# linkedin/spark-tfrecord

Hardware: AMD Instinct MI355X
Metric: rows/sec read+write (1M-row Example round-trip) (higher is better)
Workload: dtype wire(int64/float32/bytes); 1 GPU; model=Example{id:int64, ints:Int64List[8], floats:FloatList[16], tokens:BytesList[2]}, global_batch=1000000, parallelism=dp1, rows_per_rank=1000000, engine=gpu, storage=/dev/shm, crc_verify=True

## Files before the change

csrc/hip/kernels.hip:

```cpp

#include <hip/hip_runtime.h>
#include <pybind11/pybind11.h>
#include <pybind11/stl.h>
#include <rocprim/rocprim.hpp>

#include <fcntl.h>
#include <sys/mman.h>
#include <sys/stat.h>
#include <unistd.h>

#include <cstdint>
#include <map>
#include <mutex>
#include <stdexcept>
#include <string>
#include <vector>

#include "../codec_core.h"

namespace py = pybind11;
using namespace tfrec;

#define HIP_CHECK(expr)                                                          \
  do {                                                                           \
    hipError_t _e = (expr);                                                      \
    if (_e != hipSuccess)                                                        \
      throw std::runtime_error(std::string("HIP error: ") +                      \
                               hipGetErrorString(_e) + " at " __FILE__ ":" +     \
                               std::to_string(__LINE__));                        \
  } while (0)

namespace {

constexpr int kBlock = 256;

__device__ inline void stage_crc_tables(uint32_t (*lds)[256]) {
  const uint32_t* src = &kCrcTables.t[0][0];
  uint32_t* dst = &lds[0][0];
  for (int i = threadIdx.x; i < 8 * 256; i += blockDim.x) dst[i] = src[i];
  __syncthreads();
}

__device__ inline void set_err(int32_t* err, int32_t code, i64 r) {
  err[0] = code;
  i64 v = r + 1;
  atomicMax(&err[1], v > 0x7FFFFFFF ? (int32_t)0x7FFFFFFF : (int32_t)v);
}


__global__ void crc_verify_kernel(const u8* __restrict__ data,
                                  const i64* __restrict__ off,
                                  const i64* __restrict__ len, i64 R,
                                  unsigned long long* err_out) {
  __shared__ uint32_t tab[8][256];
  stage_crc_tables(tab);
  for (i64 r = blockIdx.x * (i64)blockDim.x + threadIdx.x; r < R;
       r += (i64)gridDim.x * blockDim.x) {
    const u8* h = data + off[r] - 12;
    u32 len_crc, data_crc;
    __builtin_memcpy(&len_crc, h + 8, 4);
    __builtin_memcpy(&data_crc, h + 12 + len[r], 4);
    bool ok = mask_crc(crc32c_sw(h, 8, 0, tab)) == len_crc &&
              mask_crc(crc32c_sw(h + 12, (size_t)len[r], 0, tab)) == data_crc;
    if (!ok) atomicMin(err_out, (unsigned long long)(r + 1));
  }
}


static_assert(sizeof(FieldStat) == 48, "FieldStat layout shared with Python");

__global__ void scan_records_kernel(const u8* __restrict__ data,
                                    const i64* __restrict__ off,
                                    const i64* __restrict__ len, i64 R, int32_t fmt,
                                    const u8* __restrict__ schema_blob, int F,
                                    FieldStat* __restrict__ stats,
                                    int32_t* __restrict__ err,
                                    unsigned long long* crc_err) {
  __shared__ uint32_t tab[8][256];
  if (crc_err) stage_crc_tables(tab);
  SchemaView schema = schema_view(schema_blob);
  for (i64 r = blockIdx.x * (i64)blockDim.x + threadIdx.x; r < R;
       r += (i64)gridDim.x * blockDim.x) {
    FieldStat* st = stats + r * F;
    for (int f = 0; f < F; ++f) field_stat_clear(&st[f]);
    int32_t rc;
    if (crc_err) {
      u32 payload_crc = 0;
      rc = scan_record_fused(data, off[r], len[r], fmt, schema, st,
                             &payload_crc, tab);
      if (rc == ERR_RETRY_UNFUSED) {
        for (int f = 0; f < F; ++f) field_stat_clear(&st[f]);
        rc = scan_record(data, off[r], len[r], fmt, schema, st);
        payload_crc = crc32c_sw(data + off[r], (size_t)len[r], 0, tab);
      }
      if (rc != ERR_OK)
        payload_crc = crc32c_sw(data + off[r], (size_t)len[r], 0, tab);
      const u8* h = data + off[r] - 12;
      u32 len_crc, data_crc;
      __builtin_memcpy(&len_crc, h + 8, 4);
      __builtin_memcpy(&data_crc, h + 12 + len[r], 4);
      bool ok = mask_crc(crc32c_sw(h, 8, 0, tab)) == len_crc &&
                mask_crc(payload_crc) == data_crc;
      if (!ok) atomicMin(crc_err, (unsigned long long)(r + 1));
    } else {
      rc = scan_record(data, off[r], len[r], fmt, schema, st);
    }
    if (rc != ERR_OK) set_err(err, rc, r);
    for (int f = 0; f < F; ++f)
      if (st[f].err != ERR_OK) set_err(err, st[f].err, r);
  }
}


struct DevFieldDst {
  int32_t kind;
  int32_t is_seq;
  i64* i64_vals;
  float* f32_vals;
  u8* bytes_data;
  i64* elem_len;
  i64* sub_count;
  const i64* val_base;
  const i64* byte_base;
  const i64* list_base;
};

__global__ void extract_fields_kernel(const u8* __restrict__ data, i64 R, int F,
                                      const FieldStat* __restrict__ stats,
                                      const DevFieldDst* __restrict__ metas,
                                      int32_t* __restrict__ err) {
  i64 total = R * F;
  for (i64 idx = blockIdx.x * (i64)blockDim.x + threadIdx.x; idx < total;
       idx += (i64)gridDim.x * blockDim.x) {
    i64 r = idx / F;
    int f = (int)(idx - r * F);
    const DevFieldDst& m = metas[f];
    const FieldStat& st = stats[r * F + f];
    DecodeDst dst{m.i64_vals, m.f32_vals, m.bytes_data, m.elem_len, m.sub_count};
    int32_t rc = extract_field(data, st.pos, st.len, m.kind, m.is_seq, dst,
                               m.val_base ? m.val_base[r] : 0,
                               m.byte_base ? m.byte_base[r] : 0,
                               m.list_base ? m.list_base[r] : 0);
    if (rc != ERR_OK) set_err(err, rc, r);
  }
}



__global__ void size_records_kernel(const FieldColumn* __restrict__ cols,
                                    const u8* __restrict__ schema_blob, int32_t fmt,
                                    i64 R, i64* __restrict__ psize) {
  SchemaView schema = schema_view(schema_blob);
  for (i64 r = blockIdx.x * (i64)blockDim.x + threadIdx.x; r < R;
       r += (i64)gridDim.x * blockDim.x) {
    psize[r] = record_payload_size(cols, schema, fmt, r) + kFrameOverhead;
  }
}

__global__ void emit_records_kernel(const FieldColumn* __restrict__ cols,
                                    const u8* __restrict__ schema_blob, int32_t fmt,
                                    i64 r0, i64 R, const i64* __restrict__ frame_off,
                                    u8* __restrict__ file,
                                    int32_t* __restrict__ err) {
  __shared__ uint32_t tab[8][256];
  stage_crc_tables(tab);
  SchemaView schema = schema_view(schema_blob);
  for (i64 r = r0 + blockIdx.x * (i64)blockDim.x + threadIdx.x; r < R;
       r += (i64)gridDim.x * blockDim.x) {
    i64 payload = (frame_off[r + 1] - frame_off[r]) - kFrameOverhead;
    u8* o = file + frame_off[r] + 12;
    u32 crc = 0;
    i64 emitted = emit_record_payload_fused(o, cols, schema, fmt, r, &crc,
                                            tab);
    if (emitted != payload) set_err(err, ERR_OVERFLOW, r);
    write_frame_header_footer_crc(file, frame_off[r], payload, crc, tab);
  }
}


constexpr i64 kWaveRecordBytes = 8 << 10;

__device__ inline u32 crc32c_wave(const u8* p, i64 n,
                                  const uint32_t (*tab)[256]) {
  int lane = threadIdx.x & 63;
  i64 chunk = (n + 63) / 64;
  if (chunk < 64) chunk = 64;
  i64 s = (i64)lane * chunk;
  i64 e = s + chunk < n ? s + chunk : n;
  u32 my = (s < e) ? crc32c_sw(p + s, (size_t)(e - s), 0, tab) : 0;
  u32 acc = __shfl(my, 0);
  if (chunk < n) {
    u32 op = crc32c_shift_elem((u64)chunk);
    for (int i = 1; i < 64; ++i) {
      i64 si = (i64)i * chunk;
      if (si >= n) break;
      u32 ci = __shfl(my, i);
      i64 li = (si + chunk < n ? chunk : n - si);
      acc = (li == chunk) ? (crc_gfmul(acc, op) ^ ci)
                          : crc32c_combine_fast(acc, ci, (u64)li);
    }
  }
  return acc;
}

__device__ inline void copy_wave(u8* d, const u8* s, i64 n) {
  int lane = threadIdx.x & 63;
  i64 i = (i64)lane * 8;
  for (; i + 8 <= n; i += 64 * 8) {
    u64 w;
    __builtin_memcpy(&w, s + i, 8);
    __builtin_memcpy(d + i, &w, 8);
  }
  i64 tail = n & ~((i64)7);
  for (i64 b = tail + lane; b < n; b += 64) d[b] = s[b];
}

__global__ void crc_verify_wave_kernel(const u8* __restrict__ data,
                                       const i64* __restrict__ off,
                                       const i64* __restrict__ len, i64 R,
                                       unsigned long long* err_out) {
  __shared__ uint32_t tab[8][256];
  stage_crc_tables(tab);
  i64 wave = (blockIdx.x * (i64)blockDim.x + threadIdx.x) / 64;
  i64 nwaves = ((i64)gridDim.x * blockDim.x) / 64;
  for (i64 r = wave; r < R; r += nwaves) {
    const u8* h = data + off[r] - 12;
    u32 payload = crc32c_wave(h + 12, len[r], tab);
    if ((threadIdx.x & 63) == 0) {
      u32 len_crc, data_crc;
      __builtin_memcpy(&len_crc, h + 8, 4);
      __builtin_memcpy(&data_crc, h + 12 + len[r], 4);
      bool ok = mask_crc(crc32c_sw(h, 8, 0, tab)) == len_crc &&
                mask_crc(payload) == data_crc;
      if (!ok) atomicMin(err_out, (unsigned long long)(r + 1));
    }
  }
}

__global__ void frame_bytes_wave_kernel(const u8* __restrict__ src,
                                        const i64* __restrict__ elem_off,
                                        const i64* __restrict__ frame_off, i64 R,
                                        u8* __restrict__ file) {
  __shared__ uint32_t tab[8][256];
  stage_crc_tables(tab);
  i64 wave = (blockIdx.x * (i64)blockDim.x + threadIdx.x) / 64;
  i64 nwaves = ((i64)gridDim.x * blockDim.x) / 64;
  for (i64 r = wave; r < R; r += nwaves) {
    i64 n = elem_off[r + 1] - elem_off[r];
    const u8* s = src + elem_off[r];
    u8* d = file + frame_off[r] + 12;
    copy_wave(d, s, n);
    u32 crc = crc32c_wave(s, n, tab);
    if ((threadIdx.x & 63) == 0)
      write_frame_header_footer_crc(file, frame_off[r], n, crc, tab);
  }
}

__global__ void gather_payloads_wave_kernel(const u8* __restrict__ data,
                                            const i64* __restrict__ off,
                                            const i64* __restrict__ len,
                                            const i64* __restrict__ dst_off,
                                            i64 R, u8* __restrict__ out) {
  i64 wave = (blockIdx.x * (i64)blockDim.x + threadIdx.x) / 64;
  i64 nwaves = ((i64)gridDim.x * blockDim.x) / 64;
  for (i64 r = wave; r < R; r += nwaves)
    copy_wave(out + dst_off[r], data + off[r], len[r]);
}


__device__ inline i64 wave_incl_scan(i64 v) {
  int lane = threadIdx.x & 63;
  for (int d = 1; d < 64; d <<= 1) {
    i64 y = __shfl_up(v, d);
    if (lane >= d) v += y;
  }
  return v;
}

__device__ inline i64 wave_extract_i64_packed(const u8* __restrict__ p, i64 n,
                                              i64* __restrict__ out, i64 base) {
  int lane = threadIdx.x & 63;
  i64 chunk = (n + 63) / 64;
  i64 lo = (i64)lane * chunk;
  i64 hi = lo + chunk < n ? lo + chunk : n;
  i64 cnt = 0;
  for (i64 i = lo; i < hi; ++i) cnt += !(p[i] & 0x80);
  i64 incl = wave_incl_scan(cnt);
  i64 excl = incl - cnt;
  i64 total = __shfl(incl, 63);
  i64 q = lo;
  i64 pre = 0;
  if (lo > 0 && lo < hi) {
    if (p[lo - 1] & 0x80) {
      while (q < hi && (p[q] & 0x80)) ++q;
      if (q < hi) {
        ++q;
        pre = 1;
      }
    }
  }
  i64 idx = base + excl + pre;
  while (q < hi) {
    u64 v = 0;
    int shift = 0;
    i64 j = q;
    while (j < n && shift < 70) {
      u8 b = p[j++];
      v |= (u64)(b & 0x7F) << shift;
      shift += 7;
      if (!(b & 0x80)) break;
    }
    out[idx++] = (i64)v;
    q = j;
  }
  return total;
}

__device__ inline int32_t extract_list_body_wave(const u8* __restrict__ p,
                                                 const u8* end, int32_t kind,
                                                 const DecodeDst& dst, i64* vi,
                                                 i64* bi) {
  int lane = threadIdx.x & 63;
  while (p < end) {
    u64 tag;
    p = read_varint(p, end, &tag);
    if (!p) return ERR_BAD_VARINT;
    u32 fieldno = (u32)(tag >> 3), wt = (u32)(tag & 7);
    if (fieldno != 1) {
      p = skip_field(p, end, wt);
      if (!p) return ERR_TRUNCATED;
      continue;
    }
    if (kind == KIND_BYTES) {
      u64 len;
      p = read_varint(p, end, &len);
      if (!p || (u64)(end - p) < len) return ERR_TRUNCATED;
      copy_wave(dst.bytes_data + *bi, p, (i64)len);
      if (lane == 0) dst.elem_len[*vi] = (i64)len;
      *bi += (i64)len;
      *vi += 1;
      p += len;
    } else if (kind == KIND_FLOAT) {
      if (wt == 2) {
        u64 len;
        p = read_varint(p, end, &len);
        if (!p || (u64)(end - p) < len) return ERR_TRUNCATED;
        u64 nv = len / 4;
        copy_wave((u8*)(dst.f32_vals + *vi), p, (i64)(nv * 4));
        *vi += (i64)nv;
        p += len;
      } else {
        if (end - p < 4) return ERR_TRUNCATED;
        if (lane == 0) {
          float v;
          __builtin_memcpy(&v, p, 4);
          dst.f32_vals[*vi] = v;
        }
        (*vi)++;
        p += 4;
      }
    } else {
      if (wt == 2) {
        u64 len;
        p = read_varint(p, end, &len);
        if (!p || (u64)(end - p) < len) return ERR_TRUNCATED;
        *vi += wave_extract_i64_packed(p, (i64)len, dst.i64_vals, *vi);
        p += len;
      } else {
        u64 v;
        p = read_varint(p, end, &v);
        if (!p) return ERR_BAD_VARINT;
        if (lane == 0) dst.i64_vals[*vi] = (i64)v;
        (*vi)++;
      }
    }
  }
  return ERR_OK;
}

__device__ inline int32_t extract_feature_body_wave(const u8* __restrict__ p,
                                                    const u8* end, int32_t kind,
                                                    const DecodeDst& dst,
                                                    i64* vi, i64* bi) {
  while (p < end) {
    u64 tag;
    p = read_varint(p, end, &tag);
    if (!p) return ERR_BAD_VARINT;
    u32 fieldno = (u32)(tag >> 3), wt = (u32)(tag & 7);
    if (fieldno >= 1 && fieldno <= 3 && wt == 2) {
      u64 len;
      p = read_varint(p, end, &len);
      if (!p || (u64)(end - p) < len) return ERR_TRUNCATED;
      int32_t rc = extract_list_body_wave(p, p + len, kind, dst, vi, bi);
      if (rc != ERR_OK) return rc;
      p += len;
    } else {
      p = skip_field(p, end, wt);
      if (!p) return ERR_TRUNCATED;
    }
  }
  return ERR_OK;
}

__device__ inline int32_t extract_field_wave(const u8* __restrict__ data,
                                             i64 pos, i64 len, int32_t kind,
                                             int32_t is_seq, const DecodeDst& dst,
                                             i64 val_base, i64 byte_base,
                                             i64 list_base) {
  if (pos < 0) return ERR_OK;
  int lane = threadIdx.x & 63;
  const u8* p = data + pos;
  const u8* end = p + len;
  i64 vi = val_base;
  i64 bi = byte_base;
  if (!is_seq) return extract_feature_body_wave(p, end, kind, dst, &vi, &bi);
  i64 li = list_base;
  while (p < end) {
    u64 tag;
    p = read_varint(p, end, &tag);
    if (!p) return ERR_BAD_VARINT;
    u32 fieldno = (u32)(tag >> 3), wt = (u32)(tag & 7);
    if (fieldno == 1 && wt == 2) {
      u64 flen;
      p = read_varint(p, end, &flen);
      if (!p || (u64)(end - p) < flen) return ERR_TRUNCATED;
      i64 v_before = vi;
      int32_t rc = extract_feature_body_wave(p, p + flen, kind, dst, &vi, &bi);
      if (rc != ERR_OK) return rc;
      if (lane == 0) dst.sub_count[li] = vi - v_before;
      ++li;
      p += flen;
    } else {
      p = skip_field(p, end, wt);
      if (!p) return ERR_TRUNCATED;
    }
  }
  return ERR_OK;
}

__global__ void scan_records_wave_kernel(const u8* __restrict__ data,
                                         const i64* __restrict__ off,
                                         const i64* __restrict__ len, i64 R,
                                         int32_t fmt,
                                         const u8* __restrict__ schema_blob,
                                         int F, FieldStat* __restrict__ stats,
                                         int32_t* __restrict__ err,
                                         unsigned long long* crc_err) {
  __shared__ uint32_t tab[8][256];
  stage_crc_tables(tab);
  SchemaView schema = schema_view(schema_blob);
  i64 wave = (blockIdx.x * (i64)blockDim.x + threadIdx.x) / 64;
  i64 nwaves = ((i64)gridDim.x * blockDim.x) / 64;
  int lane = threadIdx.x & 63;
  for (i64 r = wave; r < R; r += nwaves) {
    if (lane == 0) {
      FieldStat* st = stats + r * F;
      for (int f = 0; f < F; ++f) field_stat_clear(&st[f]);
      int32_t rc = scan_record(data, off[r], len[r], fmt, schema, st);
      if (rc != ERR_OK) set_err(err, rc, r);
      for (int f = 0; f < F; ++f)
        if (st[f].err != ERR_OK) set_err(err, st[f].err, r);
    }
    if (crc_err) {
      const u8* h = data + off[r] - 12;
      u32 payload = crc32c_wave(h + 12, len[r], tab);
      if (lane == 0) {
        u32 len_crc, data_crc;
        __builtin_memcpy(&len_crc, h + 8, 4);
        __builtin_memcpy(&data_crc, h + 12 + len[r], 4);
        bool ok = mask_crc(crc32c_sw(h, 8, 0, tab)) == len_crc &&
                  mask_crc(payload) == data_crc;
        if (!ok) atomicMin(crc_err, (unsigned long long)(r + 1));
      }
    }
  }
}

__global__ void extract_fields_wave_kernel(const u8* __restrict__ data, i64 R,
                                           int F,
                                           const FieldStat* __restrict__ stats,
                                           const DevFieldDst* __restrict__ metas,
                                           int32_t* __restrict__ err) {
  i64 total = R * F;
  i64 wave = (blockIdx.x * (i64)blockDim.x + threadIdx.x) / 64;
  i64 nwaves = ((i64)gridDim.x * blockDim.x) / 64;
  for (i64 idx = wave; idx < total; idx += nwaves) {
    i64 r = idx / F;
    int f = (int)(idx - r * F);
    const DevFieldDst& m = metas[f];
    const FieldStat& st = stats[r * F + f];
    DecodeDst dst{m.i64_vals, m.f32_vals, m.bytes_data, m.elem_len, m.sub_count};
    int32_t rc = extract_field_wave(data, st.pos, st.len, m.kind, m.is_seq, dst,
                                    m.val_base ? m.val_base[r] : 0,
                                    m.byte_base ? m.byte_base[r] : 0,
                                    m.list_base ? m.list_base[r] : 0);
    if (rc != ERR_OK && (threadIdx.x & 63) == 0) set_err(err, rc, r);
  }
}


__device__ inline i64 wave_emit_i64_packed(u8* __restrict__ o,
                                           const i64* __restrict__ vals,
                                           i64 v0, i64 v1) {
  int lane = threadIdx.x & 63;
  i64 n = v1 - v0;
  i64 chunk = (n + 63) / 64;
  i64 lo = v0 + (i64)lane * chunk;
  i64 hi = lo + chunk < v1 ? lo + chunk : v1;
  i64 sz = 0;
  for (i64 v = lo; v < hi; ++v) sz += varint_size((u64)vals[v]);
  i64 incl = wave_incl_scan(sz);
  u8* q = o + (incl - sz);
  for (i64 v = lo; v < hi; ++v) q = write_varint(q, (u64)vals[v]);
  return __shfl(incl, 63);
}

struct WaveCur {
  u8* base;
  i64 pos;
};

__device__ inline void wvc_put(WaveCur& w, u8 b) {
  if ((threadIdx.x & 63) == 0) w.base[w.pos] = b;
  w.pos += 1;
}

__device__ inline void wvc_varint(WaveCur& w, u64 v) {
  if ((threadIdx.x & 63) == 0) write_varint(w.base + w.pos, v);
  w.pos += varint_size(v);
}

__device__ inline void wvc_bytes(WaveCur& w, const u8* s, i64 n) {
  copy_wave(w.base + w.pos, s, n);
  w.pos += n;
}

__device__ inline void wvc_list_body(WaveCur& w, const FieldColumn& c, i64 v0,
                                     i64 v1) {
  if (c.kind == KIND_FLOAT) {
    i64 n = v1 - v0;
    if (n) {
      wvc_put(w, 0x0A);
      wvc_varint(w, (u64)(4 * n));
      wvc_bytes(w, (const u8*)(c.f32_vals + v0), 4 * n);
    }
  } else if (c.kind == KIND_INT64) {
    i64 packed = 0;
    for (i64 v = v0; v < v1; ++v) packed += varint_size((u64)c.i64_vals[v]);
    if (packed) {
      wvc_put(w, 0x0A);
      wvc_varint(w, (u64)packed);
      w.pos += wave_emit_i64_packed(w.base + w.pos, c.i64_vals, v0, v1);
    }
  } else {
    for (i64 v = v0; v < v1; ++v) {
      i64 b0 = c.elem_off[v];
      i64 blen = c.elem_off[v + 1] - b0;
      wvc_put(w, 0x0A);
      wvc_varint(w, (u64)blen);
      wvc_bytes(w, c.bytes_data + b0, blen);
    }
  }
}

__device__ inline void wvc_feature_body(WaveCur& w, const FieldColumn& c,
                                        i64 v0, i64 v1) {
  i64 body = list_body_size(c, v0, v1);
  wvc_put(w, (u8)((c.kind << 3) | 2));
  wvc_varint(w, (u64)body);
  wvc_list_body(w, c, v0, v1);
}

__device__ inline void wvc_features_entry(WaveCur& w, const FieldColumn& c,
                                          const SchemaView& s, int f, i64 v0,
                                          i64 v1) {
  i64 fb = feature_body_size(c, v0, v1);
  i64 klen = s.name_len(f);
  wvc_put(w, 0x0A);
  wvc_varint(w, (u64)klen);
  wvc_bytes(w, s.name(f), klen);
  wvc_put(w, 0x12);
  wvc_varint(w, (u64)fb);
  wvc_feature_body(w, c, v0, v1);
}

__device__ inline void wvc_feature_lists_entry(WaveCur& w, const FieldColumn& c,
                                               const SchemaView& s, int f,
                                               i64 r) {
  i64 flb = feature_list_body_size(c, r);
  i64 klen = s.name_len(f);
  wvc_put(w, 0x0A);
  wvc_varint(w, (u64)klen);
  wvc_bytes(w, s.name(f), klen);
  wvc_put(w, 0x12);
  wvc_varint(w, (u64)flb);
  for (i64 j = c.list_off[r]; j < c.list_off[r + 1]; ++j) {
    i64 fb = feature_body_size(c, c.sub_off[j], c.sub_off[j + 1]);
    wvc_put(w, 0x0A);
    wvc_varint(w, (u64)fb);
    wvc_feature_body(w, c, c.sub_off[j], c.sub_off[j + 1]);
  }
}

__device__ inline i64 emit_record_payload_wave(u8* o, const FieldColumn* cols,
                                               const SchemaView& s, int32_t fmt,
                                               i64 r) {
  i64 ctx_body = 0, fl_body = 0;
  for (int f = 0; f < s.nfields; ++f) {
    const FieldColumn& c = cols[f];
    if (!c.presence[r]) continue;
    if (!c.is_seq) {
      i64 e = features_entry_size(c, s, f, c.row_off[r], c.row_off[r + 1]);
      ctx_body += 1 + varint_size((u64)e) + e;
    } else {
      i64 e = feature_lists_entry_size(c, s, f, r);
      fl_body += 1 + varint_size((u64)e) + e;
    }
  }
  WaveCur w{o, 0};
  auto emit_ctx = [&]() {
    for (int f = 0; f < s.nfields; ++f) {
      const FieldColumn& c = cols[f];
      if (!c.presence[r] || c.is_seq) continue;
      i64 e = features_entry_size(c, s, f, c.row_off[r], c.row_off[r + 1]);
      wvc_put(w, 0x0A);
      wvc_varint(w, (u64)e);
      wvc_features_entry(w, c, s, f, c.row_off[r], c.row_off[r + 1]);
    }
  };
  auto emit_fl = [&]() {
    for (int f = 0; f < s.nfields; ++f) {
      const FieldColumn& c = cols[f];
      if (!c.presence[r] || !c.is_seq) continue;
      i64 e = feature_lists_entry_size(c, s, f, r);
      wvc_put(w, 0x0A);
      wvc_varint(w, (u64)e);
      wvc_feature_lists_entry(w, c, s, f, r);
    }
  };
  if (fmt == FMT_EXAMPLE) {
    wvc_put(w, 0x0A);
    wvc_varint(w, (u64)ctx_body);
    emit_ctx();
  } else {
    if (ctx_body) {
      wvc_put(w, 0x0A);
      wvc_varint(w, (u64)ctx_body);
      emit_ctx();
    }
    wvc_put(w, 0x12);
    wvc_varint(w, (u64)fl_body);
    emit_fl();
  }
  return w.pos;
}

__global__ void emit_records_wave_kernel(const FieldColumn* __restrict__ cols,
                                         const u8* __restrict__ schema_blob,
                                         int32_t fmt, i64 r0, i64 R,
                                         const i64* __restrict__ frame_off,
                                         u8* __restrict__ file,
                                         int32_t* __restrict__ err) {
  __shared__ uint32_t tab[8][256];
  stage_crc_tables(tab);
  SchemaView schema = schema_view(schema_blob);
  i64 wave = (blockIdx.x * (i64)blockDim.x + threadIdx.x) / 64;
  i64 nwaves = ((i64)gridDim.x * blockDim.x) / 64;
  int lane = threadIdx.x & 63;
  for (i64 r = r0 + wave; r < R; r += nwaves) {
    i64 payload = (frame_off[r + 1] - frame_off[r]) - kFrameOverhead;
    u8* o = file + frame_off[r] + 12;
    i64 emitted = emit_record_payload_wave(o, cols, schema, fmt, r);
    if (emitted != payload && lane == 0) set_err(err, ERR_OVERFLOW, r);
    __threadfence_block();
    u32 crc = crc32c_wave(o, payload, tab);
    if (lane == 0)
      write_frame_header_footer_crc(file, frame_off[r], payload, crc, tab);
  }
}

__global__ void frame_bytes_kernel(const u8* __restrict__ src,
                                   const i64* __restrict__ elem_off,
                                   const i64* __restrict__ frame_off, i64 R,
                                   u8* __restrict__ file) {
  __shared__ uint32_t tab[8][256];
  stage_crc_tables(tab);
  for (i64 r = blockIdx.x * (i64)blockDim.x + threadIdx.x; r < R;
       r += (i64)gridDim.x * blockDim.x) {
    i64 n = elem_off[r + 1] - elem_off[r];
    WriteCur w;
    wcur_init(w, file + frame_off[r] + 12, tab);
    wcur_bytes(w, src + elem_off[r], n);
    u32 crc = wcur_finish(w);
    write_frame_header_footer_crc(file, frame_off[r], n, crc, tab);
  }
}

__device__ inline u32 crc8b_reg(u64 w, const uint32_t (*tab)[256]) {
  w ^= 0xFFFFFFFFull;
  u32 c = tab[7][w & 0xFF] ^ tab[6][(w >> 8) & 0xFF] ^ tab[5][(w >> 16) & 0xFF] ^
          tab[4][(w >> 24) & 0xFF] ^ tab[3][(w >> 32) & 0xFF] ^
          tab[2][(w >> 40) & 0xFF] ^ tab[1][(w >> 48) & 0xFF] ^
          tab[0][(w >> 56) & 0xFF];
  return ~c;
}

constexpr int kPosPerLane = 16;

template <typename F>
__device__ inline void eval_frame_chunk(const u8* __restrict__ data,
                                        const u64* __restrict__ wdata, i64 N,
                                        i64 c, i64 pos_start, i64 pos_end,
                                        const uint32_t (*tab)[256], F&& f) {
  i64 p0 = c * kPosPerLane;
  i64 w0 = p0 >> 3;
  u64 w[4];
  if (p0 + 32 <= N) {
#pragma unroll
    for (int j = 0; j < 4; ++j) w[j] = wdata[w0 + j];
  } else {
#pragma unroll
    for (int j = 0; j < 4; ++j) {
      u64 v = 0;
      i64 boff = (w0 + j) * 8;
      for (int b = 0; b < 8 && boff + b < N; ++b)
        v |= (u64)data[boff + b] << (8 * b);
      w[j] = v;
    }
  }
#pragma unroll
  for (int k = 0; k < kPosPerLane; ++k) {
    i64 i = p0 + k;
    if (i + 16 > N || i >= pos_end) break;
    if (i < pos_start) continue;
    constexpr int _ppl = kPosPerLane;
    static_assert(_ppl == 16, "index math below assumes 16 positions");
    const int wi = k >> 3;
    const int sh = (k & 7) * 8;
    u64 len = (sh == 0) ? w[wi] : (w[wi] >> sh) | (w[wi + 1] << (64 - sh));
    if (len > (u64)(N - i) - 16) continue;
    const int wi2 = (k + 8) >> 3;
    const int sh2 = sh;
    u64 hi = (sh2 == 0) ? w[wi2]
                        : (w[wi2] >> sh2) | (w[wi2 + 1] << (64 - sh2));
    u32 want = (u32)hi;
    if (mask_crc(crc8b_reg(len, tab)) != want) continue;
    f(i, (i64)len);
  }
}

template <bool EMIT>
__global__ void frame_scan_pass_kernel(const u8* __restrict__ data, i64 N,
                                       i64 pos_start, i64 pos_end,
                                       i64 block_base,
                                       i64* __restrict__ block_data,
                                       i64* __restrict__ cand_pos,
                                       i64* __restrict__ cand_len) {
  __shared__ uint32_t tab[8][256];
  __shared__ unsigned int cnt[256];
  stage_crc_tables(tab);
  const u64* wdata = reinterpret_cast<const u64*>(data);
  i64 c_lo = pos_start / kPosPerLane;
  i64 c_hi = (pos_end + kPosPerLane - 1) / kPosPerLane;
  i64 c = c_lo + (i64)blockIdx.x * blockDim.x + threadIdx.x;
  unsigned int my = 0;
  if (c < c_hi)
    eval_frame_chunk(data, wdata, N, c, pos_start, pos_end, tab,
                     [&](i64, i64) { ++my; });
  cnt[threadIdx.x] = my;
  __syncthreads();
  if (!EMIT) {
    for (int off = blockDim.x / 2; off; off >>= 1) {
      if ((int)threadIdx.x < off) cnt[threadIdx.x] += cnt[threadIdx.x + off];
      __syncthreads();
    }
    if (threadIdx.x == 0) block_data[block_base + blockIdx.x] = (i64)cnt[0];
    return;
  }
  for (int off = 1; off < (int)blockDim.x; off <<= 1) {
    unsigned int v = (int)threadIdx.x >= off ? cnt[threadIdx.x - off] : 0;
    __syncthreads();
    cnt[threadIdx.x] += v;
    __syncthreads();
  }
  i64 slot = block_data[block_base + blockIdx.x] + (i64)(cnt[threadIdx.x] - my);
  if (c < c_hi)
    eval_frame_chunk(data, wdata, N, c, pos_start, pos_end, tab,
                     [&](i64 i, i64 len) {
                       cand_pos[slot] = i;
                       cand_len[slot] = len;
                       ++slot;
                     });
}


struct InferSlot {
  unsigned long long hash;
  long long nameref;
  long long code;
};
static_assert(sizeof(InferSlot) == 24, "layout shared with Python [S,3] i64");

__device__ inline u64 fnv1a64(const u8* s, u64 n) {
  u64 h = 1469598103934665603ull;
  for (u64 i = 0; i < n; ++i) h = (h ^ s[i]) * 1099511628211ull;
  return h ? h : 1ull;
}

constexpr int kLdsInfer = 64;

struct LdsInferSlot {
  unsigned long long hash;
  long long nameref;
  unsigned int code;
};

__device__ inline bool lds_infer_merge(LdsInferSlot* ltab, u64 hash,
                                       long long nameref, int code) {
  int idx = (int)(hash % (u64)kLdsInfer);
  for (int probe = 0; probe < kLdsInfer; ++probe) {
    LdsInferSlot& s = ltab[idx];
    unsigned long long seen =
        atomicCAS(&s.hash, 0ull, (unsigned long long)hash);
    if (seen == 0ull) s.nameref = nameref;
    if (seen == 0ull || seen == hash) {
      atomicMax(&s.code, (unsigned int)code);
      return true;
    }
    idx = (idx + 1) % kLdsInfer;
  }
  return false;
}

__device__ inline bool infer_slot_merge(InferSlot* table, int lo, int half,
                                        u64 hash, long long nameref, int code) {
  int idx = lo + (int)(hash % (u64)half);
  for (int probe = 0; probe < half; ++probe) {
    InferSlot& s = table[idx];
    unsigned long long seen =
        atomicCAS(&s.hash, 0ull, (unsigned long long)hash);
    if (seen == 0ull) s.nameref = nameref;
    if (seen == 0ull || seen == hash) {
      atomicMax((unsigned long long*)&s.code, (unsigned long long)code);
      return true;
    }
    idx = (idx + 1 - lo) % half + lo;
  }
  return false;
}

__device__ inline int32_t infer_features_body_dev(const u8* data, const u8* p,
                                                  const u8* end, bool seq,
                                                  LdsInferSlot* ltab,
                                                  InferSlot* table, int nslots) {
  int half = nslots / 2;
  int lo = seq ? half : 0;
  while (p < end) {
    u64 tag;
    p = read_varint(p, end, &tag);
    if (!p) return ERR_BAD_VARINT;
    u32 fieldno = (u32)(tag >> 3), wt = (u32)(tag & 7);
    if (fieldno != 1 || wt != 2) {
      p = skip_field(p, end, wt);
      if (!p) return ERR_TRUNCATED;
      continue;
    }
    u64 entry_len;
    p = read_varint(p, end, &entry_len);
    if (!p || (u64)(end - p) < entry_len) return ERR_TRUNCATED;
    const u8* ep = p;
    const u8* ee = p + entry_len;
    p = ee;
    const u8* key = nullptr;
    u64 key_len = 0;
    const u8* val = nullptr;
    u64 val_len = 0;
    while (ep < ee) {
      u64 etag;
      ep = read_varint(ep, ee, &etag);
      if (!ep) return ERR_BAD_VARINT;
      u32 efn = (u32)(etag >> 3), ewt = (u32)(etag & 7);
      if (efn == 1 && ewt == 2) {
        ep = read_varint(ep, ee, &key_len);
        if (!ep || (u64)(ee - ep) < key_len) return ERR_TRUNCATED;
        key = ep;
        ep += key_len;
      } else if (efn == 2 && ewt == 2) {
        ep = read_varint(ep, ee, &val_len);
        if (!ep || (u64)(ee - ep) < val_len) return ERR_TRUNCATED;
        val = ep;
        ep += val_len;
      } else {
        ep = skip_field(ep, ee, ewt);
        if (!ep) return ERR_TRUNCATED;
      }
    }
    if (!key) continue;
    int code = 0;
    if (val) {
      if (!seq) {
        int32_t kf = 0;
        i64 nvals = 0, nbytes = 0;
        int32_t rc = scan_feature_body(val, val + val_len, -1, &kf, &nvals, &nbytes);
        if (rc != ERR_OK) return rc;
        if (kf != 0 && nvals > 0) code = (4 - kf) + (nvals > 1 ? 3 : 0);
      } else {
        const u8* lp = val;
        const u8* le = val + val_len;
        int kind_seen = 0;
        while (lp < le) {
          u64 ltag;
          lp = read_varint(lp, le, &ltag);
          if (!lp) return ERR_BAD_VARINT;
          u32 lfn = (u32)(ltag >> 3), lwt = (u32)(ltag & 7);
          if (lfn == 1 && lwt == 2) {
            u64 flen;
            lp = read_varint(lp, le, &flen);
            if (!lp || (u64)(le - lp) < flen) return ERR_TRUNCATED;
            int32_t kf = 0;
            i64 nvals = 0, nbytes = 0;
            int32_t rc = scan_feature_body(lp, lp + flen, -1, &kf, &nvals, &nbytes);
            if (rc != ERR_OK) return rc;
            if (kf) {
              int r = 4 - kf;
              kind_seen = kind_seen > r ? kind_seen : r;
            }
            lp += flen;
          } else {
            lp = skip_field(lp, le, lwt);
            if (!lp) return ERR_TRUNCATED;
          }
        }
        if (kind_seen) code = 6 + kind_seen;
      }
    }
    if (key_len > 0xFFFF) return ERR_NAME_TOO_LONG;
    long long nameref = ((long long)(key - data) << 16) | (long long)key_len;
    u64 hash = fnv1a64(key, key_len);
    if (!lds_infer_merge(ltab, hash, nameref, code) &&
        !infer_slot_merge(table, lo, half, hash, nameref, code))
      return ERR_OVERFLOW;
  }
  return ERR_OK;
}

__global__ void infer_codes_kernel(const u8* __restrict__ data,
                                   const i64* __restrict__ off,
                                   const i64* __restrict__ len, i64 R, int32_t fmt,
                                   InferSlot* __restrict__ table, int nslots,
                                   int32_t* __restrict__ err) {
  __shared__ LdsInferSlot lctx[kLdsInfer];
  __shared__ LdsInferSlot lseq[kLdsInfer];
  for (int i = threadIdx.x; i < kLdsInfer; i += blockDim.x) {
    lctx[i].hash = 0;
    lctx[i].code = 0;
    lseq[i].hash = 0;
    lseq[i].code = 0;
  }
  __syncthreads();
  for (i64 r = blockIdx.x * (i64)blockDim.x + threadIdx.x; r < R;
       r += (i64)gridDim.x * blockDim.x) {
    const u8* p = data + off[r];
    const u8* end = p + len[r];
    while (p < end) {
      u64 tag;
      const u8* np = read_varint(p, end, &tag);
      if (!np) {
        set_err(err, ERR_BAD_VARINT, r);
        break;
      }
      p = np;
      u32 fieldno = (u32)(tag >> 3), wt = (u32)(tag & 7);
      bool is_features = fieldno == 1;
      bool is_fl = (fmt == FMT_SEQUENCE && fieldno == 2);
      if ((is_features || is_fl) && wt == 2) {
        u64 blen;
        p = read_varint(p, end, &blen);
        if (!p || (u64)(end - p) < blen) {
          set_err(err, ERR_TRUNCATED, r);
          break;
        }
        int32_t rc = infer_features_body_dev(data, p, p + blen, is_fl,
                                             is_fl ? lseq : lctx, table, nslots);
        if (rc != ERR_OK) {
          set_err(err, rc, r);
          break;
        }
        p += blen;
      } else {
        p = skip_field(p, end, wt);
        if (!p) {
          set_err(err, ERR_TRUNCATED, r);
          break;
        }
      }
    }
  }
  __syncthreads();
  int half = nslots / 2;
  for (int i = threadIdx.x; i < kLdsInfer; i += blockDim.x) {
    if (lctx[i].hash &&
        !infer_slot_merge(table, 0, half, lctx[i].hash, lctx[i].nameref,
                          (int)lctx[i].code))
      err[0] = ERR_OVERFLOW;
    if (lseq[i].hash &&
        !infer_slot_merge(table, half, half, lseq[i].hash, lseq[i].nameref,
                          (int)lseq[i].code))
      err[0] = ERR_OVERFLOW;
  }
}

__global__ void gather_payloads_kernel(const u8* __restrict__ data,
                                       const i64* __restrict__ off,
                                       const i64* __restrict__ len,
                                       const i64* __restrict__ dst_off, i64 R,
                                       u8* __restrict__ out) {
  for (i64 r = blockIdx.x * (i64)blockDim.x + threadIdx.x; r < R;
       r += (i64)gridDim.x * blockDim.x) {
    const u8* s = data + off[r];
    u8* d = out + dst_off[r];
    i64 n = len[r];
    i64 i = 0;
    for (; i + 8 <= n; i += 8) {
      u64 w;
      __builtin_memcpy(&w, s + i, 8);
      __builtin_memcpy(d + i, &w, 8);
    }
    for (; i < n; ++i) d[i] = s[i];
  }
}


inline int grid_for(i64 n) {
  i64 blocks = (n + kBlock - 1) / kBlock;
  if (blocks > 8192) blocks = 8192;
  if (blocks < 1) blocks = 1;
  return (int)blocks;
}

void gpu_crc_verify(uintptr_t data, uintptr_t off, uintptr_t len, i64 R,
                    uintptr_t err_out, uintptr_t stream, i64 avg_bytes) {
  if (avg_bytes > kWaveRecordBytes) {
    hipLaunchKernelGGL(crc_verify_wave_kernel, dim3(grid_for(R * 64)),
                       dim3(kBlock), 0, (hipStream_t)stream, (const u8*)data,
                       (const i64*)off, (const i64*)len, R,
                       (unsigned long long*)err_out);
  } else {
    hipLaunchKernelGGL(crc_verify_kernel, dim3(grid_for(R)), dim3(kBlock), 0,
                       (hipStream_t)stream, (const u8*)data, (const i64*)off,
                       (const i64*)len, R, (unsigned long long*)err_out);
  }
  HIP_CHECK(hipGetLastError());
}

void gpu_scan_records(uintptr_t data, uintptr_t off, uintptr_t len, i64 R,
                      int32_t fmt, uintptr_t schema_blob, int F, uintptr_t stats,
                      uintptr_t err, uintptr_t crc_err, uintptr_t stream,
                      i64 avg_bytes) {
  if (avg_bytes > kWaveRecordBytes) {
    hipLaunchKernelGGL(scan_records_wave_kernel, dim3(grid_for(R * 64)),
                       dim3(kBlock), 0, (hipStream_t)stream, (const u8*)data,
                       (const i64*)off, (const i64*)len, R, fmt,
                       (const u8*)schema_blob, F, (FieldStat*)stats,
                       (int32_t*)err, (unsigned long long*)crc_err);
  } else {
    hipLaunchKernelGGL(scan_records_kernel, dim3(grid_for(R)), dim3(kBlock), 0,
                       (hipStream_t)stream, (const u8*)data, (const i64*)off,
                       (const i64*)len, R, fmt, (const u8*)schema_blob, F,
                       (FieldStat*)stats, (int32_t*)err,
                       (unsigned long long*)crc_err);
  }
  HIP_CHECK(hipGetLastError());
}

void gpu_extract_fields(uintptr_t data, i64 R, int F, uintptr_t stats,
                        py::list metas, uintptr_t meta_dev, uintptr_t err,
                        uintptr_t stream, i64 avg_bytes) {
  std::vector<DevFieldDst> host_metas(F);
  for (int f = 0; f < F; ++f) {
    py::dict d = metas[f].cast<py::dict>();
    DevFieldDst& m = host_metas[f];
    m.kind = d["kind"].cast<int32_t>();
    m.is_seq = d["is_seq"].cast<int32_t>();
    m.i64_vals = (i64*)d["i64_vals"].cast<uintptr_t>();
    m.f32_vals = (float*)d["f32_vals"].cast<uintptr_t>();
    m.bytes_data = (u8*)d["bytes_data"].cast<uintptr_t>();
    m.elem_len = (i64*)d["elem_len"].cast<uintptr_t>();
    m.sub_count = (i64*)d["sub_count"].cast<uintptr_t>();
    m.val_base = (const i64*)d["val_base"].cast<uintptr_t>();
    m.byte_base = (const i64*)d["byte_base"].cast<uintptr_t>();
    m.list_base = (const i64*)d["list_base"].cast<uintptr_t>();
  }
  HIP_CHECK(hipMemcpyAsync((void*)meta_dev, host_metas.data(),
                           sizeof(DevFieldDst) * F, hipMemcpyHostToDevice,
                           (hipStream_t)stream));
  if (avg_bytes > kWaveRecordBytes) {
    hipLaunchKernelGGL(extract_fields_wave_kernel, dim3(grid_for(R * F * 64)),
                       dim3(kBlock), 0, (hipStream_t)stream, (const u8*)data,
                       R, F, (const FieldStat*)stats,
                       (const DevFieldDst*)meta_dev, (int32_t*)err);
  } else {
    hipLaunchKernelGGL(extract_fields_kernel, dim3(grid_for(R * F)),
                       dim3(kBlock), 0, (hipStream_t)stream, (const u8*)data,
                       R, F, (const FieldStat*)stats,
                       (const DevFieldDst*)meta_dev, (int32_t*)err);
  }
  HIP_CHECK(hipGetLastError());
}

size_t gpu_devcols_bytes(int F) { return sizeof(FieldColumn) * (size_t)F; }

void fill_devcols(py::list cols, std::vector<FieldColumn>& out) {
  int F = (int)cols.size();
  out.resize(F);
  for (int f = 0; f < F; ++f) {
    py::dict d = cols[f].cast<py::dict>();
    FieldColumn& c = out[f];
    c.kind = d["kind"].cast<int32_t>();
    c.is_seq = d["is_seq"].cast<int32_t>();
    c.presence = (const u8*)d["presence"].cast<uintptr_t>();
    c.row_off = (const i64*)d["row_off"].cast<uintptr_t>();
    c.list_off = (const i64*)d["list_off"].cast<uintptr_t>();
    c.sub_off = (const i64*)d["sub_off"].cast<uintptr_t>();
    c.elem_off = (const i64*)d["elem_off"].cast<uintptr_t>();
    c.bytes_data = (const u8*)d["values_bytes"].cast<uintptr_t>();
    c.i64_vals = (const i64*)d["values_i64"].cast<uintptr_t>();
    c.f32_vals = (const float*)d["values_f32"].cast<uintptr_t>();
  }
}

void gpu_size_records(py::list cols, uintptr_t cols_dev, uintptr_t schema_blob,
                      int32_t fmt, i64 R, uintptr_t psize, uintptr_t stream) {
  static thread_local std::vector<FieldColumn> host_cols;
  fill_devcols(cols, host_cols);
  HIP_CHECK(hipMemcpyAsync((void*)cols_dev, host_cols.data(),
                           sizeof(FieldColumn) * host_cols.size(),
                           hipMemcpyHostToDevice, (hipStream_t)stream));
  hipLaunchKernelGGL(size_records_kernel, dim3(grid_for(R)), dim3(kBlock), 0,
                     (hipStream_t)stream, (const FieldColumn*)cols_dev,
                     (const u8*)schema_blob, fmt, R, (i64*)psize);
  HIP_CHECK(hipGetLastError());
}

void gpu_emit_records(uintptr_t cols_dev, uintptr_t schema_blob, int32_t fmt,
                      i64 r0, i64 R, uintptr_t frame_off, uintptr_t file,
                      uintptr_t err, uintptr_t stream, i64 avg_bytes) {
  if (avg_bytes > kWaveRecordBytes) {
    hipLaunchKernelGGL(emit_records_wave_kernel, dim3(grid_for((R - r0) * 64)),
                       dim3(kBlock), 0, (hipStream_t)stream,
                       (const FieldColumn*)cols_dev, (const u8*)schema_blob,
                       fmt, r0, R, (const i64*)frame_off, (u8*)file,
                       (int32_t*)err);
  } else {
    hipLaunchKernelGGL(emit_records_kernel, dim3(grid_for(R - r0)),
                       dim3(kBlock), 0, (hipStream_t)stream,
                       (const FieldColumn*)cols_dev, (const u8*)schema_blob,
                       fmt, r0, R, (const i64*)frame_off, (u8*)file,
                       (int32_t*)err);
  }
  HIP_CHECK(hipGetLastError());
}

void gpu_frame_bytes(uintptr_t src, uintptr_t elem_off, uintptr_t frame_off, i64 R,
                     uintptr_t file, uintptr_t stream, i64 avg_bytes) {
  if (avg_bytes > kWaveRecordBytes) {
    hipLaunchKernelGGL(frame_bytes_wave_kernel, dim3(grid_for(R * 64)),
                       dim3(kBlock), 0, (hipStream_t)stream, (const u8*)src,
                       (const i64*)elem_off, (const i64*)frame_off, R,
                       (u8*)file);
  } else {
    hipLaunchKernelGGL(frame_bytes_kernel, dim3(grid_for(R)), dim3(kBlock), 0,
                       (hipStream_t)stream, (const u8*)src, (const i64*)elem_off,
                       (const i64*)frame_off, R, (u8*)file);
  }
  HIP_CHECK(hipGetLastError());
}

i64 gpu_frame_scan_blocks(i64 pos_start, i64 pos_end) {
  i64 c_lo = pos_start / kPosPerLane;
  i64 c_hi = (pos_end + kPosPerLane - 1) / kPosPerLane;
  i64 n = c_hi - c_lo;
  return (n + kBlock - 1) / kBlock;
}

void gpu_frame_scan_count(uintptr_t data, i64 N, i64 pos_start, i64 pos_end,
                          i64 block_base, uintptr_t block_counts,
                          uintptr_t stream) {
  i64 B = gpu_frame_scan_blocks(pos_start, pos_end);
  if (B <= 0) return;
  hipLaunchKernelGGL(frame_scan_pass_kernel<false>, dim3((uint32_t)B),
                     dim3(kBlock), 0, (hipStream_t)stream, (const u8*)data, N,
                     pos_start, pos_end, block_base, (i64*)block_counts,
                     nullptr, nullptr);
  HIP_CHECK(hipGetLastError());
}

void gpu_frame_scan_emit(uintptr_t data, i64 N, i64 pos_start, i64 pos_end,
                         i64 block_base, uintptr_t block_off,
                         uintptr_t cand_pos, uintptr_t cand_len,
                         uintptr_t stream) {
  i64 B = gpu_frame_scan_blocks(pos_start, pos_end);
  if (B <= 0) return;
  hipLaunchKernelGGL(frame_scan_pass_kernel<true>, dim3((uint32_t)B),
                     dim3(kBlock), 0, (hipStream_t)stream, (const u8*)data, N,
                     pos_start, pos_end, block_base, (i64*)block_off,
                     (i64*)cand_pos, (i64*)cand_len);
  HIP_CHECK(hipGetLastError());
}

void gpu_infer_codes(uintptr_t data, uintptr_t off, uintptr_t len, i64 R,
                     int32_t fmt, uintptr_t table, int nslots, uintptr_t err,
                     uintptr_t stream) {
  hipLaunchKernelGGL(infer_codes_kernel, dim3(grid_for(R)), dim3(kBlock), 0,
                     (hipStream_t)stream, (const u8*)data, (const i64*)off,
                     (const i64*)len, R, fmt, (InferSlot*)table, nslots,
                     (int32_t*)err);
  HIP_CHECK(hipGetLastError());
}

void gpu_gather_payloads(uintptr_t data, uintptr_t off, uintptr_t len,
                         uintptr_t dst_off, i64 R, uintptr_t out,
                         uintptr_t stream, i64 avg_bytes) {
  if (avg_bytes > kWaveRecordBytes) {
    hipLaunchKernelGGL(gather_payloads_wave_kernel, dim3(grid_for(R * 64)),
                       dim3(kBlock), 0, (hipStream_t)stream, (const u8*)data,
                       (const i64*)off, (const i64*)len, (const i64*)dst_off,
                       R, (u8*)out);
  } else {
    hipLaunchKernelGGL(gather_payloads_kernel, dim3(grid_for(R)), dim3(kBlock),
                       0, (hipStream_t)stream, (const u8*)data,
                       (const i64*)off, (const i64*)len, (const i64*)dst_off,
                       R, (u8*)out);
  }
  HIP_CHECK(hipGetLastError());
}


struct StridedLoadI64 {
  const i64* p;
  i64 stride;
  __host__ __device__ i64 operator()(i64 i) const { return p[i * stride]; }
};

size_t gpu_scan_temp_bytes(i64 n) {
  size_t bytes = 0;
  auto it = rocprim::make_transform_iterator(
      rocprim::make_counting_iterator<i64>(0), StridedLoadI64{nullptr, 1});
  (void)rocprim::inclusive_scan(nullptr, bytes, it, (i64*)nullptr, (size_t)n,
                                rocprim::plus<i64>());
  return bytes;
}


struct Seg3 {
  i64 v0, v1, v2;
  u32 flag;
};

struct Seg3Combine {
  __host__ __device__ Seg3 operator()(const Seg3& a, const Seg3& b) const {
    if (b.flag) return b;
    return Seg3{a.v0 + b.v0, a.v1 + b.v1, a.v2 + b.v2, a.flag};
  }
};

struct Seg3Load {
  const i64* stats;
  i64 R;
  int F;
  __host__ __device__ Seg3 operator()(i64 idx) const {
    i64 f = idx / R;
    i64 r = idx - f * R;
    const i64* st = stats + (r * F + f) * 6;
    return Seg3{st[2], st[3], st[4], r == 0 ? 1u : 0u};
  }
};

struct Seg3OutRef {
  i64* o0;
  i64* o1;
  i64* o2;
  __host__ __device__ Seg3OutRef& operator=(const Seg3& v) {
    *o0 = v.v0;
    *o1 = v.v1;
    *o2 = v.v2;
    return *this;
  }
};

struct Seg3OutIt {
  using value_type = Seg3;
  using reference = Seg3OutRef;
  using pointer = Seg3OutRef*;
  using difference_type = i64;
  using iterator_category = std::random_access_iterator_tag;
  i64* b0;
  i64* b1;
  i64* b2;
  i64 R;
  i64 pos;
  __host__ __device__ Seg3OutRef operator*() const { return (*this)[0]; }
  __host__ __device__ Seg3OutRef operator[](i64 k) const {
    i64 idx = pos + k;
    i64 f = idx / R;
    i64 r = idx - f * R;
    i64 at = f * (R + 1) + r + 1;
    return Seg3OutRef{b0 + at, b1 + at, b2 + at};
  }
  __host__ __device__ Seg3OutIt operator+(i64 k) const {
    return Seg3OutIt{b0, b1, b2, R, pos + k};
  }
  __host__ __device__ Seg3OutIt& operator+=(i64 k) {
    pos += k;
    return *this;
  }
  __host__ __device__ Seg3OutIt& operator++() {
    ++pos;
    return *this;
  }
};

size_t gpu_stat_scan_temp_bytes(i64 R, int F) {
  size_t bytes = 0;
  auto in = rocprim::make_transform_iterator(
      rocprim::make_counting_iterator<i64>(0), Seg3Load{nullptr, R, F});
  Seg3OutIt out{nullptr, nullptr, nullptr, R, 0};
  (void)rocprim::inclusive_scan(nullptr, bytes, in, out, (size_t)(R * F),
                                Seg3Combine());
  return bytes;
}

void gpu_stat_scans(uintptr_t temp, size_t temp_bytes, uintptr_t stats, i64 R,
                    int F, uintptr_t val_base, uintptr_t byte_base,
                    uintptr_t list_base, uintptr_t stream) {
  auto s = (hipStream_t)stream;
  if (R <= 0 || F <= 0) return;
  auto in = rocprim::make_transform_iterator(
      rocprim::make_counting_iterator<i64>(0),
      Seg3Load{(const i64*)stats, R, F});
  Seg3OutIt out{(i64*)val_base, (i64*)byte_base, (i64*)list_base, R, 0};
  size_t tb = temp_bytes;
  HIP_CHECK(rocprim::inclusive_scan((void*)temp, tb, in, out,
                                    (size_t)(R * F), Seg3Combine(), s));
}

void gpu_excl_sum_strided(uintptr_t temp, size_t temp_bytes, uintptr_t in,
                          i64 stride, uintptr_t out, i64 n, uintptr_t stream) {
  auto s = (hipStream_t)stream;
  HIP_CHECK(hipMemsetAsync((void*)out, 0, sizeof(i64), s));
  if (n <= 0) return;
  auto it = rocprim::make_transform_iterator(
      rocprim::make_counting_iterator<i64>(0), StridedLoadI64{(const i64*)in, stride});
  size_t tb = temp_bytes;
  hipError_t e = rocprim::inclusive_scan((void*)temp, tb, it, (i64*)out + 1,
                                         (size_t)n, rocprim::plus<i64>(), s);
  HIP_CHECK(e);
}


struct MappedFile {
  void* ptr = nullptr;
  size_t n = 0;
  dev_t dev = 0;
  ino_t ino = 0;
  bool pinned = false;
  bool writable = false;
};

std::map<std::string, MappedFile> g_mmap_cache;
std::mutex g_mmap_mu;
size_t g_mmap_bytes = 0;
constexpr size_t kMmapCacheCap = 4ull << 30;

void drop_mapping_locked(const std::string& key) {
  auto it = g_mmap_cache.find(key);
  if (it == g_mmap_cache.end()) return;
  if (it->second.pinned) {
    (void)hipDeviceSynchronize();
    (void)hipHostUnregister(it->second.ptr);
  }
  munmap(it->second.ptr, it->second.n);
  g_mmap_bytes -= it->second.n;
  g_mmap_cache.erase(it);
}

void sweep_stale_locked() {
  for (auto it = g_mmap_cache.begin(); it != g_mmap_cache.end();) {
    struct stat st {};
    bool live = stat(it->first.c_str(), &st) == 0 &&
                st.st_dev == it->second.dev && st.st_ino == it->second.ino &&
                (size_t)st.st_size >= it->second.n;
    if (live) {
      ++it;
    } else {
      auto key = it->first;
      ++it;
      drop_mapping_locked(key);
    }
  }
}

py::tuple file_mmap_pinned(const std::string& path, i64 n, bool writable) {
  if (n <= 0) return py::make_tuple((uintptr_t)0, true);
  std::lock_guard<std::mutex> lk(g_mmap_mu);
  sweep_stale_locked();
  int flags = writable ? (O_RDWR | O_CREAT) : O_RDWR;
  int fd = ::open(path.c_str(), flags, 0644);
  bool rdonly = false;
  if (fd < 0 && !writable) {
    fd = ::open(path.c_str(), O_RDONLY);
    rdonly = true;
  }
  if (fd < 0)
    throw std::runtime_error("open failed: " + path + ": " + strerror(errno));
  struct stat st {};
  if (fstat(fd, &st) != 0) {
    ::close(fd);
    throw std::runtime_error("stat failed: " + path);
  }
  auto it = g_mmap_cache.find(path);
  if (it != g_mmap_cache.end()) {
    MappedFile& m = it->second;
    if (m.dev == st.st_dev && m.ino == st.st_ino && m.n == (size_t)n &&
        st.st_size >= (off_t)n && (m.writable || !writable)) {
      ::close(fd);
      return py::make_tuple((uintptr_t)m.ptr, m.pinned);
    }
    drop_mapping_locked(path);
  }
  if (writable && st.st_size != (off_t)n && ftruncate(fd, (off_t)n) != 0) {
    int e = errno;
    ::close(fd);
    throw std::runtime_error("ftruncate failed: " + path + ": " + strerror(e));
  }
  if (!writable && st.st_size < (off_t)n) {
    ::close(fd);
    throw std::runtime_error("short file: " + path);
  }
  while (g_mmap_bytes + (size_t)n > kMmapCacheCap && !g_mmap_cache.empty())
    drop_mapping_locked(g_mmap_cache.begin()->first);
  int prot = PROT_READ | ((writable || !rdonly) ? PROT_WRITE : 0);
  void* p = mmap(nullptr, (size_t)n, prot, MAP_SHARED, fd, 0);
  ::close(fd);
  if (p == MAP_FAILED)
    throw std::runtime_error("mmap failed: " + path + ": " + strerror(errno));
  bool pinned = hipHostRegister(p, (size_t)n, hipHostRegisterDefault) == hipSuccess;
  if (!pinned) (void)hipGetLastError();
  MappedFile m{p, (size_t)n, st.st_dev, st.st_ino, pinned,
               writable || !rdonly};
  g_mmap_cache[path] = m;
  g_mmap_bytes += (size_t)n;
  return py::make_tuple((uintptr_t)p, pinned);
}

void file_mmap_drop(const std::string& path) {
  std::lock_guard<std::mutex> lk(g_mmap_mu);
  drop_mapping_locked(path);
}

void file_mmap_sync(const std::string& path) {
  std::lock_guard<std::mutex> lk(g_mmap_mu);
  auto it = g_mmap_cache.find(path);
  if (it != g_mmap_cache.end() && it->second.ptr) {
    if (msync(it->second.ptr, it->second.n, MS_SYNC) != 0)
      throw std::runtime_error("msync failed: " + path + ": " +
                               strerror(errno));
  }
  int fd = ::open(path.c_str(), O_RDONLY);
  if (fd >= 0) {
    (void)fsync(fd);
    ::close(fd);
  }
}


void gpu_memcpy_d2h(uintptr_t dst, uintptr_t src, i64 n, uintptr_t stream) {
  HIP_CHECK(hipMemcpyAsync((void*)dst, (const void*)src, (size_t)n,
                           hipMemcpyDeviceToHost, (hipStream_t)stream));
}

void gpu_memcpy_h2d(uintptr_t dst, uintptr_t src, i64 n, uintptr_t stream) {
  HIP_CHECK(hipMemcpyAsync((void*)dst, (const void*)src, (size_t)n,
                           hipMemcpyHostToDevice, (hipStream_t)stream));
}

}

void register_gpu(py::module_& m) {
  m.def("gpu_device_count", []() {
    int n = 0;
    hipError_t e = hipGetDeviceCount(&n);
    return (e == hipSuccess) ? n : -static_cast<int>(e);
  });
  m.def("gpu_crc_verify", &gpu_crc_verify, py::arg("data"), py::arg("off"),
        py::arg("len"), py::arg("R"), py::arg("err_out"), py::arg("stream"),
        py::arg("avg_bytes") = 0);
  m.def("gpu_scan_records", &gpu_scan_records, py::arg("data"), py::arg("off"),
        py::arg("len"), py::arg("R"), py::arg("fmt"), py::arg("schema_blob"),
        py::arg("F"), py::arg("stats"), py::arg("err"), py::arg("crc_err"),
        py::arg("stream"), py::arg("avg_bytes") = 0);
  m.def("gpu_extract_fields", &gpu_extract_fields, py::arg("data"),
        py::arg("R"), py::arg("F"), py::arg("stats"), py::arg("metas"),
        py::arg("meta_dev"), py::arg("err"), py::arg("stream"),
        py::arg("avg_bytes") = 0);
  m.def("gpu_size_records", &gpu_size_records);
  m.def("gpu_emit_records", &gpu_emit_records, py::arg("cols_dev"),
        py::arg("schema_blob"), py::arg("fmt"), py::arg("r0"), py::arg("R"),
        py::arg("frame_off"), py::arg("file"), py::arg("err"),
        py::arg("stream"), py::arg("avg_bytes") = 0);
  m.def("gpu_frame_bytes", &gpu_frame_bytes, py::arg("src"),
        py::arg("elem_off"), py::arg("frame_off"), py::arg("R"),
        py::arg("file"), py::arg("stream"), py::arg("avg_bytes") = 0);
  m.def("gpu_frame_scan_blocks", &gpu_frame_scan_blocks);
  m.def("gpu_frame_scan_count", &gpu_frame_scan_count);
  m.def("gpu_frame_scan_emit", &gpu_frame_scan_emit);
  m.def("gpu_gather_payloads", &gpu_gather_payloads, py::arg("data"),
        py::arg("off"), py::arg("len"), py::arg("dst_off"), py::arg("R"),
        py::arg("out"), py::arg("stream"), py::arg("avg_bytes") = 0);
  m.def("gpu_infer_codes", &gpu_infer_codes);
  m.def("gpu_scan_temp_bytes", &gpu_scan_temp_bytes);
  m.def("gpu_stat_scan_temp_bytes", &gpu_stat_scan_temp_bytes);
  m.def("gpu_stat_scans", &gpu_stat_scans);
  m.def("gpu_excl_sum_strided", &gpu_excl_sum_strided);
  m.def("file_mmap_pinned", &file_mmap_pinned, py::arg("path"), py::arg("n"),
        py::arg("writable"));
  m.def("file_mmap_drop", &file_mmap_drop);
  m.def("file_mmap_sync", &file_mmap_sync);
  m.def("gpu_memcpy_d2h", &gpu_memcpy_d2h);
  m.def("gpu_memcpy_h2d", &gpu_memcpy_h2d);
  m.def("gpu_devcols_bytes", &gpu_devcols_bytes);
  m.def("gpu_devmeta_bytes", []() { return sizeof(DevFieldDst); });
  m.def("gpu_fieldstat_words", []() { return sizeof(FieldStat) / 8; });
}
```

spark_tfrecord_amd/engine/gpu.py:

```python

from __future__ import annotations

import os
from typing import List, Optional

import numpy as np
import torch

from .. import _native
from ..columnar import RecordBatch, WireColumn, schema_blob, wire_fields
from ..schema import KIND_BYTES, KIND_FLOAT, KIND_INT64, StructType, is_sequence_field, wire_kind_of

FMT = {"Example": _native.FMT_EXAMPLE, "SequenceExample": _native.FMT_SEQUENCE}

_U64_MAX = 0xFFFFFFFFFFFFFFFF


def _stream() -> int:
    return torch.cuda.current_stream().cuda_stream


def _dev(x, dtype, device="cuda") -> torch.Tensor:
    if isinstance(x, torch.Tensor):
        return x.to(device=device, dtype=dtype).contiguous()
    arr = np.ascontiguousarray(x)
    import warnings

    with warnings.catch_warnings():
        warnings.simplefilter("ignore", UserWarning)
        return torch.as_tensor(arr, dtype=dtype).to(device)


def check_native():
    if not getattr(_native, "HAS_GPU_KERNELS", False):
        raise RuntimeError("_native was built without HIP kernels; rebuild "
                           "with build_native.py before using the GPU engine")



import threading as _threading

_pinned_tls = _threading.local()


def pinned_buffer(tag: str, nbytes: int) -> torch.Tensor:
    pool = getattr(_pinned_tls, "pool", None)
    if pool is None:
        pool = _pinned_tls.pool = {}
    buf = pool.get(tag)
    if buf is None or buf.numel() < nbytes:
        cap = max(nbytes, int((buf.numel() if buf is not None else 1 << 20) * 1.5))
        buf = torch.empty(cap, dtype=torch.uint8, pin_memory=True)
        pool[tag] = buf
    return buf


_CHUNK = 64 << 20
_READ_SLICE = int(os.environ.get("TFREC_READ_SLICE", 48 << 20))
_WRITE_SLICES = int(os.environ.get("TFREC_WRITE_SLICES", 8))
_PRESCAN = os.environ.get("TFREC_PRESCAN", "0") == "1"
_SYNC_WRITES = os.environ.get("TFREC_SYNC", "1") != "0"


def read_file_to_device(path: str, device="cuda") -> torch.Tensor:
    import os as _os

    n = _os.path.getsize(path)
    dev_t = torch.empty(max(n, 1), dtype=torch.uint8, device=device)[:n]
    if n:
        ptr, pinned = _native.file_mmap_pinned(path, n, False)
        if pinned:
            _multi_dma(dev_t.data_ptr(), ptr, n, _native.gpu_memcpy_h2d,
                       after_main=True)
            return dev_t
    return _read_file_staged(path, dev_t)


_copy_streams: Optional[list] = None


def _dma_streams() -> list:
    global _copy_streams
    if _copy_streams is None:
        _copy_streams = [torch.cuda.Stream() for _ in range(2)]
    return _copy_streams


def _multi_dma(dst: int, src: int, n: int, fn, after_main: bool):
    streams = _dma_streams()
    main = torch.cuda.current_stream()
    k = min(len(streams), max(1, n // (16 << 20)))
    span = (n + k - 1) // k
    for i in range(k):
        o = i * span
        m = min(span, n - o)
        s = streams[i]
        s.wait_stream(main)
        fn(dst + o, src + o, m, s.cuda_stream)
    if after_main:
        for i in range(k):
            main.wait_stream(streams[i])
    else:
        for i in range(k):
            streams[i].synchronize()


def _read_file_staged(path: str, dev: torch.Tensor) -> torch.Tensor:
    import os as _os

    n = dev.numel()
    buf = pinned_buffer("fread", min(n, 2 * _CHUNK) or 1)
    ev = [torch.cuda.Event(), torch.cuda.Event()]
    fd = _os.open(path, _os.O_RDONLY)
    try:
        pos = 0
        which = 0
        while pos < n:
            m = min(_CHUNK, n - pos)
            ev[which].synchronize()
            _native.pread_parallel(fd, buf.data_ptr() + which * _CHUNK, m, pos)
            dev[pos:pos + m].copy_(buf[which * _CHUNK:which * _CHUNK + m],
                                   non_blocking=True)
            ev[which].record()
            pos += m
            which ^= 1 if n > _CHUNK else 0
    finally:
        _os.close(fd)
    return dev


def device_to_file(img: torch.Tensor, path: str):
    import os as _os

    n = img.numel()
    if n == 0:
        open(path, "wb").close()
        return
    ptr, pinned = _native.file_mmap_pinned(path, n, True)
    if pinned:
        _multi_dma(ptr, img.data_ptr(), n, _native.gpu_memcpy_d2h,
                   after_main=False)
        if _SYNC_WRITES:
            _native.file_mmap_sync(path)
        return
    _write_file_staged(img, path)


def _write_file_staged(img: torch.Tensor, path: str):
    import os as _os

    n = img.numel()
    buf = pinned_buffer("fwrite", min(n, 2 * _CHUNK) or 1)
    ev = [torch.cuda.Event(), torch.cuda.Event()]
    fd = _os.open(path, _os.O_RDWR | _os.O_CREAT, 0o644)
    try:
        pos = 0
        which = 0
        m0 = min(_CHUNK, n)
        if n:
            buf[0:m0].copy_(img[0:m0], non_blocking=True)
            ev[0].record()
        while pos < n:
            m = min(_CHUNK, n - pos)
            nxt = pos + m
            nwhich = which ^ (1 if n > _CHUNK else 0)
            if nxt < n:
                m2 = min(_CHUNK, n - nxt)
                buf[nwhich * _CHUNK:nwhich * _CHUNK + m2].copy_(
                    img[nxt:nxt + m2], non_blocking=True)
                ev[nwhich].record()
            ev[which].synchronize()
            _native.pwrite_parallel(fd, buf.data_ptr() + which * _CHUNK, m, pos)
            pos = nxt
            which = nwhich
        _os.ftruncate(fd, n)
        if _SYNC_WRITES:
            _os.fsync(fd)
    finally:
        _os.close(fd)



_scan_ws = {}


def _scan_workspace(n: int, device) -> torch.Tensor:
    key = (device.index if hasattr(device, "index") else 0)
    need = _native.gpu_scan_temp_bytes(max(n, 1))
    ws = _scan_ws.get(key)
    if ws is None or ws.numel() < need:
        ws = torch.empty(int(need * 2), dtype=torch.uint8, device=device)
        _scan_ws[key] = ws
    return ws


def _excl_sum_into(out_ptr: int, in_ptr: int, stride: int, n: int, device):
    ws = _scan_workspace(n, device)
    _native.gpu_excl_sum_strided(ws.data_ptr(), ws.numel(), in_ptr, stride,
                                 out_ptr, n, _stream())


def excl_sum(t: torch.Tensor) -> torch.Tensor:
    n = t.numel()
    out = torch.empty(n + 1, dtype=torch.int64, device=t.device)
    _excl_sum_into(out.data_ptr(), t.data_ptr(), 1, n, t.device)
    return out


def device_to_bytes(img: torch.Tensor) -> bytes:
    n = img.numel()
    buf = pinned_buffer("d2h", n)
    buf[:n].copy_(img, non_blocking=True)
    torch.cuda.synchronize()
    return buf.numpy()[:n].tobytes()


def device_to_pinned_view(img: torch.Tensor, tag: str = "d2h_img") -> np.ndarray:
    n = img.numel()
    buf = pinned_buffer(tag, n)
    buf[:n].copy_(img, non_blocking=True)
    torch.cuda.synchronize()
    return buf.numpy()[:n]



def scan_frames_device(data: torch.Tensor):
    check_native()
    N = data.numel()
    device = data.device
    if N == 0:
        z = torch.zeros(0, dtype=torch.int64, device=device)
        return z, z.clone()
    B = _native.gpu_frame_scan_blocks(0, N)
    block_counts = torch.empty(B, dtype=torch.int64, device=device)
    _native.gpu_frame_scan_count(data.data_ptr(), N, 0, N, 0,
                                 block_counts.data_ptr(), _stream())
    off, lens, _ = _emit_and_chain(data, [(0, N)], block_counts, N)
    return off, lens


def _prescan_prefix(data, pre_ranges, block_counts, nblocks, N, arrived,
                    schema, record_type):
    device = data.device
    nb_pre = sum(nblocks[:len(pre_ranges)])
    if nb_pre == 0:
        return None
    block_off = excl_sum(block_counts[:nb_pre])
    C = int(block_off[-1].item())
    if C == 0:
        return None
    pos = torch.empty(C, dtype=torch.int64, device=device)
    lens = torch.empty(C, dtype=torch.int64, device=device)
    base = 0
    for s, e in pre_ranges:
        _native.gpu_frame_scan_emit(data.data_ptr(), N, s, e, base,
                                    block_off.data_ptr(), pos.data_ptr(),
                                    lens.data_ptr(), _stream())
        base += _native.gpu_frame_scan_blocks(s, e)
    K = int(torch.searchsorted(pos + 16 + lens, torch.tensor(
        arrived + 1, device=device)).item())
    if K == 0:
        return None
    fields = wire_fields(schema)
    F = len(fields)
    if F == 0:
        return None
    blob = torch.frombuffer(bytearray(schema_blob(schema)),
                            dtype=torch.uint8).to(device)
    stats1 = torch.empty((K, F, 6), dtype=torch.int64, device=device)
    err1 = torch.zeros(2, dtype=torch.int32, device=device)
    off1 = (pos[:K] + 12).contiguous()
    lens1 = lens[:K].contiguous()
    _native.gpu_scan_records(data.data_ptr(), off1.data_ptr(),
                             lens1.data_ptr(), K, FMT[record_type],
                             blob.data_ptr(), F, stats1.data_ptr(),
                             err1.data_ptr(), 0, _stream())
    return stats1, err1, K


def _emit_and_chain(data, ranges, block_counts, N):
    device = data.device
    block_off = excl_sum(block_counts)
    C = int(block_off[-1].item())
    if C == 0:
        raise RuntimeError("corrupt TFRecord: no valid frame header found")
    pos = torch.empty(C, dtype=torch.int64, device=device)
    lens = torch.empty(C, dtype=torch.int64, device=device)
    base = 0
    for s, e in ranges:
        _native.gpu_frame_scan_emit(data.data_ptr(), N, s, e, base,
                                    block_off.data_ptr(), pos.data_ptr(),
                                    lens.data_ptr(), _stream())
        base += _native.gpu_frame_scan_blocks(s, e)
    expect_next = pos + 16 + lens
    ok = bool(((pos[0] == 0) & (expect_next[-1] == N)
               & (expect_next[:-1] == pos[1:]).all()).item())
    if not ok:
        pos_h = pos.cpu().numpy()
        len_h = lens.cpu().numpy()
        import numpy as _np

        keep = []
        cur = 0
        idx = 0
        pmap = {int(p): i for i, p in enumerate(pos_h)}
        while cur < N:
            i = pmap.get(cur)
            if i is None:
                raise RuntimeError(
                    f"corrupt TFRecord: broken frame chain at offset {cur}")
            keep.append(i)
            cur = int(pos_h[i] + 16 + len_h[i])
        sel = torch.as_tensor(_np.asarray(keep, _np.int64), device=device)
        pos = pos[sel]
        lens = lens[sel]
    return pos + 12, lens, ok



def crc_verify_device(data: torch.Tensor, off: torch.Tensor, lens: torch.Tensor,
                      avg_bytes: int = 0):
    R = off.numel()
    if R == 0:
        return
    if not avg_bytes:
        avg_bytes = max(0, (data.numel() // R) - 16)
    err = torch.full((1,), -1, dtype=torch.int64, device=data.device)
    _native.gpu_crc_verify(data.data_ptr(), off.data_ptr(), lens.data_ptr(), R,
                           err.data_ptr(), _stream(), avg_bytes)
    bad = int(err.item())
    if bad != -1:
        raise RuntimeError(
            f"corrupt TFRecord: bad CRC in record {bad - 1 if bad > 0 else bad}")


def decode_device(data: torch.Tensor, off: torch.Tensor, lens: torch.Tensor,
                  schema: StructType, record_type: str,
                  verify_crc: bool = True, prescan=None) -> RecordBatch:
    check_native()
    device = data.device
    R = off.numel()
    fields = wire_fields(schema)
    F = len(fields)
    if verify_crc and record_type == "ByteArray":
        crc_verify_device(data, off, lens)

    if record_type == "ByteArray":
        dst_off = excl_sum(lens.contiguous())
        total = int(dst_off[-1].item())
        out = torch.empty(total, dtype=torch.uint8, device=device)
        if R:
            _native.gpu_gather_payloads(data.data_ptr(), off.data_ptr(),
                                        lens.data_ptr(), dst_off.data_ptr(), R,
                                        out.data_ptr(), _stream(), total // R)
        col = WireColumn(kind=KIND_BYTES, is_seq=False,
                         presence=torch.ones(R, dtype=torch.uint8, device=device),
                         row_off=torch.arange(R + 1, dtype=torch.int64, device=device),
                         values=out, elem_off=dst_off)
        return RecordBatch(schema, [col], R)

    if F == 0 or R == 0:
        cols = [WireColumn(wire_kind_of(f.dataType), is_sequence_field(f.dataType),
                           torch.zeros(R, dtype=torch.uint8, device=device),
                           torch.zeros(R + 1, dtype=torch.int64, device=device),
                           torch.zeros(0, dtype=torch.int64, device=device))
                for f in fields]
        return RecordBatch(schema, cols, R)

    blob = torch.frombuffer(bytearray(schema_blob(schema)),
                            dtype=torch.uint8).to(device)
    stats = torch.empty((R, F, 6), dtype=torch.int64, device=device)
    err = torch.zeros(2, dtype=torch.int32, device=device)
    crc_err = None
    fuse_crc = verify_crc
    if fuse_crc:
        crc_err = torch.full((1,), -1, dtype=torch.int64, device=device)
    r0 = 0
    err1 = None
    if prescan is not None:
        stats1, err1, K = prescan
        if K <= R and stats1.shape[1] == F:
            stats[:K].copy_(stats1)
            r0 = K
        else:
            err1 = None
    avg_bytes = max(0, (data.numel() // R) - 16) if R else 0
    if R > r0:
        stride = F * 6 * 8
        _native.gpu_scan_records(data.data_ptr(), off.data_ptr() + r0 * 8,
                                 lens.data_ptr() + r0 * 8, R - r0,
                                 FMT[record_type], blob.data_ptr(), F,
                                 stats.data_ptr() + r0 * stride,
                                 err.data_ptr(),
                                 crc_err.data_ptr() if fuse_crc else 0,
                                 _stream(), avg_bytes)
    crc_err_pre = None
    if fuse_crc and r0 > 0:
        crc_err_pre = torch.full((1,), -1, dtype=torch.int64, device=device)
        _native.gpu_crc_verify(data.data_ptr(), off.data_ptr(),
                               lens.data_ptr(), r0, crc_err_pre.data_ptr(),
                               _stream(), 0)

    val_base = torch.empty((F, R + 1), dtype=torch.int64, device=device)
    byte_base = torch.empty((F, R + 1), dtype=torch.int64, device=device)
    list_base = torch.empty((F, R + 1), dtype=torch.int64, device=device)
    val_base[:, 0] = 0
    byte_base[:, 0] = 0
    list_base[:, 0] = 0
    key = ("stat", device.index if hasattr(device, "index") else 0)
    need = _native.gpu_stat_scan_temp_bytes(R, F)
    ws = _scan_ws.get(key)
    if ws is None or ws.numel() < need:
        ws = torch.empty(int(need * 2) or 1, dtype=torch.uint8, device=device)
        _scan_ws[key] = ws
    _native.gpu_stat_scans(ws.data_ptr(), ws.numel(), stats.data_ptr(), R, F,
                           val_base.data_ptr(), byte_base.data_ptr(),
                           list_base.data_ptr(), _stream())
    totals = torch.stack([val_base[:, -1], byte_base[:, -1], list_base[:, -1]])
    totals_h = totals.cpu()
    if fuse_crc:
        bad = int(crc_err.item())
        bad_abs = (bad - 1 + r0) if bad != -1 else -1
        if crc_err_pre is not None:
            bp = int(crc_err_pre.item())
            if bp != -1:
                bad_abs = bp - 1 if bad_abs == -1 else min(bad_abs, bp - 1)
        if bad_abs != -1:
            raise RuntimeError(
                f"corrupt TFRecord: bad CRC in record {bad_abs}")
    rc = int(err[0].item())
    rec = int(err[1].item()) - 1 + r0
    if rc == 0 and err1 is not None:
        rc = int(err1[0].item())
        rec = int(err1[1].item()) - 1
    if rc != 0:
        where = f" in record {rec}" if rec >= 0 else ""
        raise RuntimeError(f"TFRecord decode failed{where} (native error "
                           f"{rc}; kind mismatch or malformed record)")

    metas = []
    outs = []
    for i, f in enumerate(fields):
        kind = wire_kind_of(f.dataType)
        seq = is_sequence_field(f.dataType)
        nv = int(totals_h[0, i])
        nb = int(totals_h[1, i])
        nl = int(totals_h[2, i])
        o = {"kind": kind, "seq": seq}
        o["i64_vals"] = torch.empty(nv if kind == KIND_INT64 else 0,
                                    dtype=torch.int64, device=device)
        o["f32_vals"] = torch.empty(nv if kind == KIND_FLOAT else 0,
                                    dtype=torch.float32, device=device)
        o["bytes_data"] = torch.empty(nb, dtype=torch.uint8, device=device)
        o["elem_len"] = torch.empty(nv if kind == KIND_BYTES else 0,
                                    dtype=torch.int64, device=device)
        o["sub_count"] = torch.empty(nl, dtype=torch.int64, device=device)
        outs.append(o)
        metas.append({
            "kind": kind, "is_seq": 1 if seq else 0,
            "i64_vals": o["i64_vals"].data_ptr(),
            "f32_vals": o["f32_vals"].data_ptr(),
            "bytes_data": o["bytes_data"].data_ptr(),
            "elem_len": o["elem_len"].data_ptr(),
            "sub_count": o["sub_count"].data_ptr(),
            "val_base": val_base[i].data_ptr(),
            "byte_base": byte_base[i].data_ptr(),
            "list_base": list_base[i].data_ptr() if seq else 0,
        })

    meta_dev = torch.empty(F * _native.gpu_devmeta_bytes(), dtype=torch.uint8,
                           device=device)
    _native.gpu_extract_fields(data.data_ptr(), R, F, stats.data_ptr(), metas,
                               meta_dev.data_ptr(), err.data_ptr(), _stream(),
                               avg_bytes)

    cols: List[WireColumn] = []
    for i, (f, o) in enumerate(zip(fields, outs)):
        kind = o["kind"]
        seq = o["seq"]
        presence = (stats[:, i, 0] >= 0).to(torch.uint8)
        elem_off = None
        if kind == KIND_BYTES:
            elem_off = excl_sum(o["elem_len"])
        sub_off = None
        if seq:
            sub_off = excl_sum(o["sub_count"])
        values = (o["i64_vals"] if kind == KIND_INT64 else
                  o["f32_vals"] if kind == KIND_FLOAT else o["bytes_data"])
        cols.append(WireColumn(kind, seq, presence, val_base[i], values,
                               elem_off, list_base[i] if seq else None, sub_off))
    if int(err[0].item()) != 0:
        rec = int(err[1].item()) - 1
        where = f" (record {rec})" if rec >= 0 else ""
        raise RuntimeError(f"TFRecord decode failed in value extraction"
                           f"{where} (native error {int(err[0].item())})")
    return RecordBatch(schema, cols, R)


def decode_buffer_device(data_np: np.ndarray, schema: StructType, record_type: str,
                         verify_crc: bool = True, device="cuda") -> RecordBatch:
    data_np = np.ascontiguousarray(data_np, np.uint8)
    n = data_np.size
    stage = pinned_buffer("h2d", n)
    stage.numpy()[:n] = data_np
    data = torch.empty(n, dtype=torch.uint8, device=device)
    data.copy_(stage[:n], non_blocking=True)
    off, lens = scan_frames_device(data)
    return decode_device(data, off, lens, schema, record_type, verify_crc)


def read_file_to_batch(path: str, schema: StructType, record_type: str,
                       verify_crc: bool = True, device="cuda") -> RecordBatch:
    return read_file_to_batch_pipelined(path, schema, record_type, verify_crc,
                                        device)



def _col_ptrs(col: WireColumn) -> dict:
    def p(t):
        return t.data_ptr() if isinstance(t, torch.Tensor) and t.numel() else 0

    return {
        "kind": col.kind, "is_seq": 1 if col.is_seq else 0,
        "presence": p(col.presence), "row_off": p(col.row_off),
        "list_off": p(col.list_off) if col.list_off is not None else 0,
        "sub_off": p(col.sub_off) if col.sub_off is not None else 0,
        "elem_off": p(col.elem_off) if col.elem_off is not None else 0,
        "values_bytes": p(col.values) if col.kind == KIND_BYTES else 0,
        "values_i64": p(col.values) if col.kind == KIND_INT64 else 0,
        "values_f32": p(col.values) if col.kind == KIND_FLOAT else 0,
    }


def _check_emit_err(err: torch.Tensor):
    if int(err[0].item()) != 0:
        rec = int(err[1].item()) - 1
        where = f" in record {rec}" if rec >= 0 else ""
        raise RuntimeError(f"TFRecord encode failed: size/emit mismatch{where}")


def encode_device(batch: RecordBatch, record_type: str) -> torch.Tensor:
    check_native()
    R = batch.num_rows
    device = batch.columns[0].presence.device if batch.columns else torch.device("cuda")
    if record_type == "ByteArray":
        col = batch.columns[0]
        lens = col.elem_off[1:] - col.elem_off[:-1]
        frame_off = excl_sum((lens + 16).contiguous())
        total = int(frame_off[-1].item())
        file = torch.empty(total, dtype=torch.uint8, device=device)
        if R:
            _native.gpu_frame_bytes(col.values.data_ptr(), col.elem_off.data_ptr(),
                                    frame_off.data_ptr(), R, file.data_ptr(),
                                    _stream(), (total // R) - 16)
        return file

    blob = torch.frombuffer(bytearray(schema_blob(batch.schema)),
                            dtype=torch.uint8).to(device)
    col_dicts = [_col_ptrs(c) for c in batch.columns]
    cols_dev = torch.empty(_native.gpu_devcols_bytes(len(col_dicts)),
                           dtype=torch.uint8, device=device)
    psize = torch.empty(R, dtype=torch.int64, device=device)
    _native.gpu_size_records(col_dicts, cols_dev.data_ptr(), blob.data_ptr(),
                             FMT[record_type], R, psize.data_ptr(), _stream())
    frame_off = excl_sum(psize)
    total = int(frame_off[-1].item())
    file = torch.empty(total, dtype=torch.uint8, device=device)
    err = torch.zeros(2, dtype=torch.int32, device=device)
    _native.gpu_emit_records(cols_dev.data_ptr(), blob.data_ptr(),
                             FMT[record_type], 0, R, frame_off.data_ptr(),
                             file.data_ptr(), err.data_ptr(), _stream(),
                             total // max(R, 1))
    _check_emit_err(err)
    return file


def write_batch_to_file(batch: RecordBatch, path: str,
                        record_type: str = "Example",
                        slices: Optional[int] = None) -> int:
    check_native()
    R = batch.num_rows
    if record_type == "ByteArray" or R == 0:
        img = encode_device(batch, record_type)
        device_to_file(img, path)
        return img.numel()
    device = batch.columns[0].presence.device
    blob = torch.frombuffer(bytearray(schema_blob(batch.schema)),
                            dtype=torch.uint8).to(device)
    col_dicts = [_col_ptrs(c) for c in batch.columns]
    cols_dev = torch.empty(_native.gpu_devcols_bytes(len(col_dicts)),
                           dtype=torch.uint8, device=device)
    psize = torch.empty(R, dtype=torch.int64, device=device)
    _native.gpu_size_records(col_dicts, cols_dev.data_ptr(), blob.data_ptr(),
                             FMT[record_type], R, psize.data_ptr(), _stream())
    frame_off = excl_sum(psize)
    S = max(1, min(slices if slices is not None else _WRITE_SLICES, R))
    ridx = [R * s // S for s in range(S + 1)]
    bounds = frame_off[ridx].cpu()
    total = int(bounds[-1])
    file = torch.empty(total, dtype=torch.uint8, device=device)
    err = torch.zeros(2, dtype=torch.int32, device=device)
    ptr, pinned = _native.file_mmap_pinned(path, total, True)
    if not pinned:
        _native.gpu_emit_records(cols_dev.data_ptr(), blob.data_ptr(),
                                 FMT[record_type], 0, R, frame_off.data_ptr(),
                                 file.data_ptr(), err.data_ptr(), _stream(),
                                 total // R)
        _check_emit_err(err)
        _write_file_staged(file, path)
        return total
    main = torch.cuda.current_stream()
    streams = _dma_streams()
    for s in range(S):
        _native.gpu_emit_records(cols_dev.data_ptr(), blob.data_ptr(),
                                 FMT[record_type], ridx[s], ridx[s + 1],
                                 frame_off.data_ptr(), file.data_ptr(),
                                 err.data_ptr(), _stream(), total // R)
        b0, b1 = int(bounds[s]), int(bounds[s + 1])
        if b1 > b0:
            w = streams[s % len(streams)]
            w.wait_stream(main)
            _native.gpu_memcpy_d2h(ptr + b0, file.data_ptr() + b0, b1 - b0,
                                   w.cuda_stream)
    for w in streams:
        w.synchronize()
    if _SYNC_WRITES:
        _native.file_mmap_sync(path)
    _check_emit_err(err)
    return total


def read_file_to_batch_pipelined(path: str, schema: StructType, record_type: str,
                                 verify_crc: bool = True,
                                 device="cuda") -> RecordBatch:
    import os as _os

    check_native()
    n = _os.path.getsize(path)
    if n == 0:
        z = torch.zeros(0, dtype=torch.int64, device=device)
        return decode_device(torch.zeros(0, dtype=torch.uint8, device=device),
                             z, z.clone(), schema, record_type, verify_crc)
    ptr, pinned = _native.file_mmap_pinned(path, n, False)
    if not pinned:
        data = _read_file_staged(path, torch.empty(n, dtype=torch.uint8,
                                                   device=device))
        off, lens = scan_frames_device(data)
        return decode_device(data, off, lens, schema, record_type, verify_crc)
    data = torch.empty(n, dtype=torch.uint8, device=device)
    span = _READ_SLICE
    S = max(1, (n + span - 1) // span)
    ranges = []
    scanned = 0
    for s in range(S):
        b1 = min(n, (s + 1) * span)
        scan_end = b1 - 32 if s < S - 1 else n
        if scan_end > scanned:
            ranges.append((scanned, scan_end))
            scanned = scan_end
    nblocks = [int(_native.gpu_frame_scan_blocks(a, b)) for a, b in ranges]
    block_counts = torch.empty(max(sum(nblocks), 1), dtype=torch.int64,
                               device=device)
    main = torch.cuda.current_stream()
    streams = _dma_streams()
    events = []
    for st in streams:
        st.wait_stream(main)
    for s in range(S):
        b0, b1 = s * span, min(n, (s + 1) * span)
        st = streams[s % len(streams)]
        _native.gpu_memcpy_h2d(data.data_ptr() + b0, ptr + b0, b1 - b0,
                               st.cuda_stream)
        ev = torch.cuda.Event()
        ev.record(st)
        events.append(ev)
    data.record_stream(streams[0])
    if len(streams) > 1:
        data.record_stream(streams[1])

    def launch_counts(ri: int, base: int):
        _native.gpu_frame_scan_count(data.data_ptr(), n, ranges[ri][0],
                                     ranges[ri][1], base,
                                     block_counts.data_ptr(), _stream())

    k0 = ((2 * S) // 3 if _PRESCAN and S >= 3 and record_type != "ByteArray"
          else 0)

    ri = 0
    base = 0

    def consume_slices(upto: int):
        nonlocal ri, base
        for s in range(upto):
            if events[s] is None:
                continue
            main.wait_event(events[s])
            events[s] = None
            scan_end = min(n, (s + 1) * span) - 32 if s < S - 1 else n
            if ri < len(ranges) and ranges[ri][1] == scan_end:
                launch_counts(ri, base)
                base += nblocks[ri]
                ri += 1

    prescan = None
    if k0:
        consume_slices(k0)
        prescan = _prescan_prefix(data, ranges[:ri], block_counts, nblocks, n,
                                  arrived=min(n, k0 * span), schema=schema,
                                  record_type=record_type)
    consume_slices(S)
    off, lens, clean = _emit_and_chain(data, ranges, block_counts, n)
    if not clean:
        prescan = None
    return decode_device(data, off, lens, schema, record_type, verify_crc,
                         prescan=prescan)


def gz_device_meta(path: str):
    from ..io import paths as P

    if not getattr(_native, "HAS_GPU_KERNELS", False):
        return None
    return P.parse_gz_segments_file(path)


def _device_inflate_group(data: torch.Tensor, gz_items, device) -> bool:
    import os as _os

    comp_sizes = [_os.path.getsize(p) for p, _, _ in gz_items]
    comp_total = sum(comp_sizes)
    comp = torch.empty(max(comp_total, 1), dtype=torch.uint8,
                       device=device)[:comp_total]
    main = torch.cuda.current_stream()
    streams = _dma_streams()
    in_off = []
    in_len = []
    out_off = []
    out_len = []
    used = []
    coff = 0
    for k, (p, meta, out_base) in enumerate(gz_items):
        body_off, segs, _crc, _isize = meta
        ptr, pinned = _native.file_mmap_pinned(p, comp_sizes[k], False)
        if pinned:
            st = streams[k % len(streams)]
            st.wait_stream(main)
            _native.gpu_memcpy_h2d(comp.data_ptr() + coff, ptr, comp_sizes[k],
                                   st.cuda_stream)
            used.append(st)
        else:
            _read_file_staged(p, comp[coff:coff + comp_sizes[k]])
        so = coff + body_off
        uo = out_base
        for c, u in segs:
            in_off.append(so)
            in_len.append(c)
            out_off.append(uo)
            out_len.append(u)
            so += c
            uo += u
        coff += comp_sizes[k]
    for st in set(used):
        main.wait_stream(st)
    meta_np = np.array([in_off, in_len, out_off, out_len], np.int64)
    force = _os.environ.get("TFREC_INFLATE_STREAMS", "")
    spw_lit = 2
    if force in ("1", "2", "4"):
        spw_lit = int(force)
        lit = np.full(meta_np.shape[1], spw_lit > 1)
    else:
        lit = meta_np[1] >= (0.85 * np.maximum(meta_np[3], 1))
    err = torch.full((1,), -1, dtype=torch.int64, device=device)
    for mask, spw in ((lit, spw_lit), (~lit, 1)):
        k = int(mask.sum())
        if k == 0:
            continue
        idx = np.nonzero(mask)[0]
        if spw == 2 and k > 2:
            idx = idx[np.argsort(-meta_np[3, idx], kind="stable")]
        sub = torch.as_tensor(
            np.ascontiguousarray(meta_np[:, idx])).to(device)
        _native.gpu_inflate_segments(
            comp.data_ptr(), sub[0].data_ptr(), sub[1].data_ptr(),
            sub[2].data_ptr(), sub[3].data_ptr(), k,
            data.data_ptr(), err.data_ptr(), _stream(), spw)
    return int(err.item()) == -1


def read_gzip_file_to_device(path: str, device="cuda") -> Optional[torch.Tensor]:
    meta = gz_device_meta(path)
    if meta is None:
        return None
    total_u = sum(u for _, u in meta[1])
    data = torch.empty(max(total_u, 1), dtype=torch.uint8,
                       device=device)[:total_u]
    if not _device_inflate_group(data, [(path, meta, 0)], device):
        return None
    return data


def read_files_to_batch(paths, schema: StructType, record_type: str,
                        verify_crc: bool = True, device="cuda"):
    import os as _os

    from ..io import paths as P

    check_native()
    metas = []
    sizes = []
    for p in paths:
        if P.codec_from_path(p) == "gzip":
            meta = P.parse_gz_segments_file(p)
            if meta is None:
                raise ValueError(f"gzip file without segment table: {p} "
                                 "(host path required)")
            metas.append(meta)
            sizes.append(sum(u for _, u in meta[1]))
        else:
            metas.append(None)
            sizes.append(_os.path.getsize(p))
    n = sum(sizes)
    if n == 0:
        if schema is None:
            raise ValueError(
                "Could not infer schema: no non-empty TFRecord files found")
        z = torch.zeros(0, dtype=torch.int64, device=device)
        return (decode_device(torch.zeros(0, dtype=torch.uint8, device=device),
                              z, z.clone(), schema, record_type, verify_crc),
                np.zeros(len(paths), np.int64))
    data = torch.empty(n, dtype=torch.uint8, device=device)
    bounds = np.zeros(len(paths) + 1, np.int64)
    np.cumsum(sizes, out=bounds[1:])
    main = torch.cuda.current_stream()
    streams = _dma_streams()
    gz_items = []
    for i, p in enumerate(paths):
        if not sizes[i]:
            continue
        if metas[i] is not None:
            gz_items.append((p, metas[i], int(bounds[i])))
            continue
        ptr, pinned = _native.file_mmap_pinned(p, sizes[i], False)
        if pinned:
            st = streams[i % len(streams)]
            _native.gpu_memcpy_h2d(data.data_ptr() + int(bounds[i]), ptr,
                                   sizes[i], st.cuda_stream)
            main.wait_stream(st)
        else:
            _read_file_staged(p, data[int(bounds[i]):int(bounds[i + 1])])
    if gz_items and not _device_inflate_group(data, gz_items, device):
        import logging

        logging.getLogger(__name__).warning(
            "device inflate rejected a segment; host zlib fallback for "
            "%d gzip file(s)", len(gz_items))
        for p, meta, base in gz_items:
            blob = np.frombuffer(P.decompress_file(p), np.uint8)
            stage = pinned_buffer("gzfb", blob.size)
            stage.numpy()[:blob.size] = blob
            data[base:base + blob.size].copy_(stage[:blob.size],
                                              non_blocking=True)
            torch.cuda.current_stream().synchronize()
    off, lens = scan_frames_device(data)
    frame_start = off - 12
    counts = torch.searchsorted(
        frame_start, torch.as_tensor(bounds, device=device)).cpu().numpy()
    row_counts = np.diff(counts)
    if schema is None:
        from ..infer import byte_array_schema, schema_from_codes

        if record_type == "ByteArray":
            schema = byte_array_schema()
        else:
            i = next((k for k in range(len(paths)) if row_counts[k] > 0), None)
            if i is None:
                raise ValueError(
                    "Could not infer schema: no non-empty TFRecord files found")
            r0, r1 = int(counts[i]), int(counts[i + 1])
            codes = infer_codes_device(data, off[r0:r1].contiguous(),
                                       lens[r0:r1].contiguous(), record_type)
            schema = schema_from_codes(codes)
    batch = decode_device(data, off, lens, schema, record_type, verify_crc)
    return batch, row_counts


def encode_partitions_device(batch: RecordBatch, part_codes: np.ndarray,
                             num_parts: int, record_type: str):
    check_native()
    R = batch.num_rows
    device = batch.columns[0].presence.device if batch.columns else torch.device("cuda")
    blob = torch.frombuffer(bytearray(schema_blob(batch.schema)),
                            dtype=torch.uint8).to(device)
    col_dicts = [_col_ptrs(c) for c in batch.columns]
    cols_dev = torch.empty(_native.gpu_devcols_bytes(len(col_dicts)),
                           dtype=torch.uint8, device=device)
    psize = torch.empty(R, dtype=torch.int64, device=device)
    _native.gpu_size_records(col_dicts, cols_dev.data_ptr(), blob.data_ptr(),
                             FMT[record_type], R, psize.data_ptr(), _stream())
    frame_off = excl_sum(psize)
    total = int(frame_off[-1].item())
    file = torch.empty(total, dtype=torch.uint8, device=device)
    err = torch.zeros(2, dtype=torch.int32, device=device)
    _native.gpu_emit_records(cols_dev.data_ptr(), blob.data_ptr(),
                             FMT[record_type], 0, R, frame_off.data_ptr(),
                             file.data_ptr(), err.data_ptr(), _stream(),
                             total // max(R, 1))
    codes = torch.as_tensor(np.ascontiguousarray(part_codes, np.int64),
                            device=device)
    order = torch.argsort(codes, stable=True)
    sizes = psize[order].contiguous()
    dst_off = excl_sum(sizes)
    src_off = frame_off[:-1][order].contiguous()
    out = torch.empty(total, dtype=torch.uint8, device=device)
    _native.gpu_gather_payloads(file.data_ptr(), src_off.data_ptr(),
                                sizes.data_ptr(), dst_off.data_ptr(), R,
                                out.data_ptr(), _stream(), total // max(R, 1))
    counts = torch.bincount(codes, minlength=num_parts)
    row_bound = torch.nn.functional.pad(torch.cumsum(counts, 0), (1, 0))
    byte_bound = dst_off[row_bound].cpu().numpy()
    _check_emit_err(err)
    ranges = [(p, int(byte_bound[p]), int(byte_bound[p + 1]))
              for p in range(num_parts) if byte_bound[p + 1] > byte_bound[p]]
    return out, ranges



_INFER_SLOTS = 2048
_INFER_SLOTS_MAX = 1 << 21
_ERR_OVERFLOW = -5
_ERR_NAME_TOO_LONG = -6


def infer_codes_device(data: torch.Tensor, off: torch.Tensor,
                       lens: torch.Tensor, record_type: str) -> dict:
    check_native()
    device = data.device
    fmt = FMT["SequenceExample" if record_type == "SequenceExample" else "Example"]
    R = off.numel()
    slots = _INFER_SLOTS
    while True:
        table = torch.zeros((slots, 3), dtype=torch.int64, device=device)
        err = torch.zeros(2, dtype=torch.int32, device=device)
        if R:
            _native.gpu_infer_codes(data.data_ptr(), off.data_ptr(),
                                    lens.data_ptr(), R, fmt, table.data_ptr(),
                                    slots, err.data_ptr(), _stream())
        tab = table.cpu().numpy()
        rc = int(err[0].item())
        if rc == _ERR_OVERFLOW:
            if slots < _INFER_SLOTS_MAX:
                slots *= 4
                continue
            raise RuntimeError(
                "schema inference failed: more than "
                f"{_INFER_SLOTS_MAX // 2} distinct feature names")
        if rc == _ERR_NAME_TOO_LONG:
            raise RuntimeError(
                "schema inference failed: a feature name exceeds 65535 bytes")
        if rc != 0:
            rec = int(err[1].item()) - 1
            where = f" (record {rec})" if rec >= 0 else ""
            raise RuntimeError(f"malformed record during schema inference"
                               f"{where} (native error {rc})")
        break
    used = np.nonzero(tab[:, 0])[0]
    if len(used) == 0:
        return {}
    refs = tab[used, 1]
    offs = (refs >> 16).astype(np.int64)
    nlens = (refs & 0xFFFF).astype(np.int64)
    lo = int(offs.min())
    hi = int((offs + nlens).max())
    codes: dict = {}
    if hi - lo <= (4 << 20):
        blob = data[lo:hi].cpu().numpy().tobytes()
        for o, ln, code in zip(offs, nlens, tab[used, 2]):
            name = blob[o - lo:o - lo + ln].decode("utf-8", errors="replace")
            codes[name] = max(codes.get(name, 0), int(code))
    else:
        for o, ln, code in zip(offs, nlens, tab[used, 2]):
            name = data[o:o + ln].cpu().numpy().tobytes().decode("utf-8", errors="replace")
            codes[name] = max(codes.get(name, 0), int(code))
    return codes


def infer_schema_file(path: str, record_type: str, device="cuda"):
    from ..infer import schema_from_codes

    data = read_file_to_device(path, device)
    off, lens = scan_frames_device(data)
    return schema_from_codes(infer_codes_device(data, off, lens, record_type))


def batch_to_device(batch: RecordBatch, device="cuda") -> RecordBatch:
    cols = []
    for c in batch.columns:
        cols.append(WireColumn(
            c.kind, c.is_seq,
            _dev(c.presence, torch.uint8, device),
            _dev(c.row_off, torch.int64, device),
            _dev(c.values, {KIND_INT64: torch.int64, KIND_FLOAT: torch.float32,
                            KIND_BYTES: torch.uint8}[c.kind], device),
            _dev(c.elem_off, torch.int64, device) if c.elem_off is not None else None,
            _dev(c.list_off, torch.int64, device) if c.list_off is not None else None,
            _dev(c.sub_off, torch.int64, device) if c.sub_off is not None else None,
        ))
    return RecordBatch(batch.schema, cols, batch.num_rows)


def batch_to_host(batch: RecordBatch) -> RecordBatch:
    streams = _dma_streams()
    main = torch.cuda.current_stream()
    state = {"used": False, "k": 0}

    def h(t):
        if not isinstance(t, torch.Tensor):
            return t
        if not t.is_cuda:
            return t.numpy()
        host = torch.empty_like(t, device="cpu", pin_memory=True)
        if not state["used"]:
            for s in streams:
                s.wait_stream(main)
            state["used"] = True
        nbytes = t.numel() * t.element_size()
        if nbytes >= (8 << 20) and t.is_contiguous() and len(streams) > 1:
            flat_d = t.view(-1)
            flat_h = host.view(-1)
            n = flat_d.numel()
            step = (n + len(streams) - 1) // len(streams)
            for i, st in enumerate(streams):
                lo = i * step
                hi = min(n, lo + step)
                if lo >= hi:
                    break
                with torch.cuda.stream(st):
                    flat_h[lo:hi].copy_(flat_d[lo:hi], non_blocking=True)
                t.record_stream(st)
            return host.numpy()
        st = streams[state["k"] % len(streams)]
        state["k"] += 1
        with torch.cuda.stream(st):
            host.copy_(t, non_blocking=True)
        t.record_stream(st)
        return host.numpy()

    cols = [WireColumn(c.kind, c.is_seq, h(c.presence), h(c.row_off), h(c.values),
                       h(c.elem_off) if c.elem_off is not None else None,
                       h(c.list_off) if c.list_off is not None else None,
                       h(c.sub_off) if c.sub_off is not None else None)
            for c in batch.columns]
    if state["used"]:
        for s in streams:
            s.synchronize()
    return RecordBatch(batch.schema, cols, batch.num_rows)



def decode_buffer_to_cpu(data_np: np.ndarray, schema: StructType, record_type: str,
                         verify_crc: bool = True) -> RecordBatch:
    return batch_to_host(decode_buffer_device(data_np, schema, record_type,
                                              verify_crc))


def encode_batch_from_cpu(batch: RecordBatch, record_type: str) -> bytes:
    dev_batch = batch_to_device(batch)
    file = encode_device(dev_batch, record_type)
    return device_to_bytes(file)
```

spark_tfrecord_amd/io/writer.py:

```python

from __future__ import annotations

import os
import uuid
from typing import Dict, List, Optional, Sequence

import numpy as np
import pyarrow as pa

from .. import engine as engine_mod
from ..arrow_interop import schema_from_arrow, schema_to_arrow, table_to_batch
from ..columnar import RecordBatch
from ..engine import cpu as cpu_engine
from ..schema import BinaryType, StructType, validate_schema_for_record_type
from ..utils import IOMetrics, StageTimer
from . import paths as P

__all__ = ["write_tfrecord", "normalize_input"]

RECORD_TYPES = ("Example", "SequenceExample", "ByteArray")


def normalize_input(data, schema: Optional[StructType]) -> pa.Table:
    if isinstance(data, dict) and schema is not None:
        target = schema_to_arrow(schema)
        for f in target:
            if f.name not in data:
                raise KeyError(f"column '{f.name}' not found in input data")
        try:
            return pa.table({f.name: data[f.name] for f in target},
                            schema=target)
        except (pa.ArrowInvalid, pa.ArrowTypeError, pa.ArrowNotImplementedError):
            pass
    if hasattr(data, "to_arrow_table"):
        table = data.to_arrow_table()
    elif isinstance(data, pa.Table):
        table = data
    elif isinstance(data, pa.RecordBatch):
        table = pa.Table.from_batches([data])
    elif hasattr(data, "__dataframe__") or str(type(data).__module__).startswith("pandas"):
        table = pa.Table.from_pandas(data, preserve_index=False)
    elif isinstance(data, dict):
        table = pa.table(data)
    elif isinstance(data, list):
        table = pa.Table.from_pylist(data)
    else:
        raise TypeError(f"Cannot write object of type {type(data).__name__}")
    if schema is not None:
        target = schema_to_arrow(schema)
        cols = []
        for f in target:
            if f.name not in table.column_names:
                raise KeyError(f"column '{f.name}' not found in input data")
            cols.append(table.column(f.name).cast(f.type))
        table = pa.table(cols, schema=target)
    return table


def _partition_dir_value(v) -> str:
    if v is None:
        return "__HIVE_DEFAULT_PARTITION__"
    if isinstance(v, float) and v == int(v):
        return str(int(v))
    s = str(v)
    return P.escape_path_name(s) if s else "__HIVE_DEFAULT_PARTITION__"


def _factorize_partitions(table: pa.Table, partition_by: Sequence[str]):
    import pyarrow.compute as pc

    idx_cols = []
    val_lists = []
    for c in partition_by:
        arr = table.column(c)
        if isinstance(arr, pa.ChunkedArray):
            arr = (arr.chunk(0) if arr.num_chunks == 1
                   else arr.combine_chunks() if arr.num_chunks
                   else pa.array([], arr.type))
        if isinstance(arr, pa.ChunkedArray):
            arr = arr.chunk(0) if arr.num_chunks else pa.array([], arr.type)
        de = arr.dictionary_encode()
        vals = de.dictionary.to_pylist()
        idx = pc.fill_null(de.indices, len(vals)).to_numpy(zero_copy_only=False)
        idx_cols.append(idx.astype(np.int64))
        val_lists.append(vals + [None])
    if len(idx_cols) == 1:
        return idx_cols[0], [(v,) for v in val_lists[0]]
    code = idx_cols[0].copy()
    for i in range(1, len(idx_cols)):
        code = code * len(val_lists[i]) + idx_cols[i]
    uniq, inv = np.unique(code, return_inverse=True)
    combos = []
    for u in uniq:
        rem = int(u)
        rev = []
        for vals in reversed(val_lists[1:]):
            rem, k = divmod(rem, len(vals))
            rev.append(vals[k])
        rev.append(val_lists[0][rem])
        combos.append(tuple(reversed(rev)))
    return inv.astype(np.int64), combos


_PIPE_CHUNK_ROWS = int(os.environ.get("TFREC_WRITE_CHUNK_ROWS", "131072"))


def _single_shard_pipelined(table: pa.Table, schema: StructType,
                            record_type: str, fpath: str, eng: str,
                            metrics: Optional[IOMetrics]):
    R = table.num_rows
    pool = P.shared_pool()
    os.makedirs(os.path.dirname(fpath), exist_ok=True)
    tmp = P.hidden_tmp_path(fpath, f"tmp.{uuid.uuid4().hex[:8]}")
    fd = os.open(tmp, os.O_CREAT | os.O_WRONLY | os.O_TRUNC, 0o644)
    nbytes = 0
    prev_write = None
    tag_futs: Dict[str, object] = {}

    def _append(view, after):
        if after is not None:
            after.result()
        mv = view if isinstance(view, bytes) else memoryview(view).cast("B")
        n = 0
        while n < len(mv):
            n += os.write(fd, mv[n:])
        return n

    try:
        for ci, lo in enumerate(range(0, R, _PIPE_CHUNK_ROWS)):
            chunk = table.slice(lo, min(_PIPE_CHUNK_ROWS, R - lo))
            batch = table_to_batch(chunk, schema)
            if eng == "gpu":
                from ..engine import gpu as gpu_engine

                img = gpu_engine.encode_device(
                    gpu_engine.batch_to_device(batch), record_type)
                tag = f"encw{ci % 2}"
                prev = tag_futs.get(tag)
                if prev is not None:
                    prev.result()
                raw = gpu_engine.device_to_pinned_view(img, tag=tag)
            else:
                tag = None
                raw = cpu_engine.encode_batch(batch, record_type)
            nbytes += len(raw) if isinstance(raw, bytes) else raw.nbytes
            if tag is None and prev_write is not None and ci % 4 == 0:
                prev_write.result()
            prev_write = pool.submit(_append, raw, prev_write)
            if tag is not None:
                tag_futs[tag] = prev_write
        if prev_write is not None:
            prev_write.result()
        os.fsync(fd)
    except BaseException:
        if prev_write is not None:
            try:
                prev_write.result()
            except BaseException:
                pass
        os.close(fd)
        try:
            os.unlink(tmp)
        except OSError:
            pass
        raise
    os.close(fd)
    os.replace(tmp, fpath)
    if metrics is not None:
        metrics.add(rows=R, nbytes=nbytes, files=1)


def _encode_and_write(table: pa.Table, schema: StructType, record_type: str,
                      out_dir: str, codec: Optional[str], job_id: str,
                      num_shards: int, shard_offset: int, eng: str,
                      metrics: Optional[IOMetrics] = None):
    from concurrent.futures import ThreadPoolExecutor

    R = table.num_rows
    bounds = np.linspace(0, R, num_shards + 1).astype(np.int64)

    def _compress_write(raw: bytes, fpath: str, rows: int):
        payload = P.compress_bytes(raw, codec)
        P.write_file_atomic(payload, fpath)
        if metrics is not None:
            metrics.add(rows=rows, nbytes=len(payload), files=1)

    if num_shards == 1:
        fpath = os.path.join(out_dir, P.part_file_name(shard_offset, codec,
                                                       job_id))
        if codec is None and R > 2 * _PIPE_CHUNK_ROWS:
            _single_shard_pipelined(table, schema, record_type, fpath, eng,
                                    metrics)
            return
        batch = table_to_batch(table, schema)
        if eng == "gpu":
            from ..engine import gpu as gpu_engine

            img = gpu_engine.encode_device(
                gpu_engine.batch_to_device(batch), record_type)
            raw = gpu_engine.device_to_pinned_view(img, tag="encw0")
        else:
            raw = cpu_engine.encode_batch(batch, record_type)
        _compress_write(raw, fpath, R)
        return

    if R < 32_768:
        for s in range(num_shards):
            lo, hi = int(bounds[s]), int(bounds[s + 1])
            if hi == lo:
                continue
            batch = table_to_batch(table.slice(lo, hi - lo), schema)
            if eng == "gpu":
                from ..engine import gpu as gpu_engine

                img = gpu_engine.encode_device(
                    gpu_engine.batch_to_device(batch), record_type)
                raw = gpu_engine.device_to_pinned_view(img, tag="encw0")
            else:
                raw = cpu_engine.encode_batch(batch, record_type)
            _compress_write(raw, os.path.join(
                out_dir, P.part_file_name(shard_offset + s, codec, job_id)),
                hi - lo)
        return

    pool = P.shared_pool()
    futs = []
    tag_futs = {}
    for s in range(num_shards):
        lo, hi = int(bounds[s]), int(bounds[s + 1])
        if num_shards > 1 and hi == lo:
            continue
        chunk = table.slice(lo, hi - lo)
        batch = table_to_batch(chunk, schema)
        fname = P.part_file_name(shard_offset + s, codec, job_id)
        fpath = os.path.join(out_dir, fname)
        if eng == "gpu":
            from ..engine import gpu as gpu_engine

            dev_batch = gpu_engine.batch_to_device(batch)
            img = gpu_engine.encode_device(dev_batch, record_type)
            tag = f"encw{s % 2}"
            prev = tag_futs.get(tag)
            if prev is not None:
                prev.result()
            raw = gpu_engine.device_to_pinned_view(img, tag=tag)
        else:
            raw = cpu_engine.encode_batch(batch, record_type)
        f = pool.submit(_compress_write, raw, fpath, hi - lo)
        if eng == "gpu":
            tag_futs[tag] = f
        futs.append(f)
    for f in futs:
        f.result()


def write_tfrecord(data, path: str, record_type: str = "Example",
                   codec: Optional[str] = None, mode: str = "errorifexists",
                   partition_by: Optional[Sequence[str]] = None,
                   schema: Optional[StructType] = None, num_shards: int = 1,
                   engine: str = "auto", write_success: bool = True,
                   shard_offset: int = 0, job_id: Optional[str] = None,
                   _apply_mode: bool = True) -> None:
    if record_type not in RECORD_TYPES:
        raise ValueError(
            f"Unsupported recordType {record_type!r} (expected one of {RECORD_TYPES})")
    codec = P.normalize_codec(codec)
    table = normalize_input(data, schema)
    if schema is None:
        schema = schema_from_arrow(table.schema)
    validate_schema_for_record_type(schema, record_type)
    eng = engine_mod.resolve_engine(engine)

    if record_type == "ByteArray":
        first = schema.fields[0]
        if not isinstance(first.dataType, BinaryType):
            raise TypeError(
                "ByteArray record type requires the first column to be BinaryType")

    if _apply_mode:
        if not P.apply_save_mode(path, mode):
            return
    if job_id is None:
        job_id = uuid.uuid4().hex[:12]
    metrics = IOMetrics("write")

    if partition_by:
        for c in partition_by:
            if c not in table.column_names:
                raise KeyError(f"partition column '{c}' not found")
        data_cols = [c for c in table.column_names if c not in set(partition_by)]
        data_schema = StructType([f for f in schema.fields if f.name in set(data_cols)])
        codes, combos = _factorize_partitions(table, partition_by)
        stripped = table.select(data_cols)

        def part_dir(combo) -> str:
            d = os.path.join(path, *(f"{c}={_partition_dir_value(v)}"
                                     for c, v in zip(partition_by, combo)))
            os.makedirs(d, exist_ok=True)
            return d

        if (eng == "gpu" and record_type != "ByteArray" and num_shards == 1
                and table.num_rows > 0):
            from ..engine import gpu as gpu_engine

            batch = gpu_engine.batch_to_device(
                table_to_batch(stripped, data_schema))
            img, ranges = gpu_engine.encode_partitions_device(
                batch, codes, len(combos), record_type)
            view = gpu_engine.device_to_pinned_view(img)

            def _write_part(p, lo, hi):
                sub_dir = part_dir(combos[p])
                fpath = os.path.join(
                    sub_dir, P.part_file_name(shard_offset, codec, job_id))
                payload = (view[lo:hi] if codec is None
                           else P.compress_bytes(view[lo:hi].tobytes(), codec))
                P.write_file_atomic(payload, fpath)
                return len(payload)

            for nb in P.shared_pool().map(lambda a: _write_part(*a), ranges):
                if metrics is not None:
                    metrics.add(nbytes=nb, files=1)
            if metrics is not None:
                metrics.add(rows=table.num_rows)
        else:
            for p, combo in enumerate(combos):
                idxs = np.nonzero(codes == p)[0]
                if idxs.size == 0:
                    continue
                sub = stripped.take(pa.array(idxs, type=pa.int64()))
                _encode_and_write(sub, data_schema, record_type, part_dir(combo),
                                  codec, job_id, num_shards, shard_offset, eng,
                                  metrics)
    else:
        _encode_and_write(table, schema, record_type, path, codec, job_id,
                          num_shards, shard_offset, eng, metrics)

    if write_success:
        P.write_success_marker(path)
    metrics.finish()
```

Before: 94.76 million rows/s.

## Stream decode per slice: scan, stat-scan and extract records while file slices arrive

Adds record-range offsets (rec_base/r0) and block caps to the scan, extract and stat-scan kernels, plus a device frame-chain kernel. The Python side gains a streaming row/value buffer manager that grows capacity incrementally, so parsing and extraction run on each slice as it lands instead of after the whole file is read. This is meant to overlap the file transfer with decode. In exchange it adds buffer regrow copies, many more small kernel launches, and block caps that can reduce per-kernel throughput. A writer change also drops duplicate partition ranges that map to the same directory.

Result: faster. 110.9 million rows/s (median of 6 runs) (+17.0%).

```diff
diff --git a/csrc/hip/kernels.hip b/csrc/hip/kernels.hip
--- a/csrc/hip/kernels.hip
+++ b/csrc/hip/kernels.hip
@@ -75,7 +75,8 @@
                                     const u8* __restrict__ schema_blob, int F,
                                     FieldStat* __restrict__ stats,
                                     int32_t* __restrict__ err,
-                                    unsigned long long* crc_err) {
+                                    unsigned long long* crc_err,
+                                    i64 rec_base) {
   __shared__ uint32_t tab[8][256];
   if (crc_err) stage_crc_tables(tab);
   SchemaView schema = schema_view(schema_blob);
@@ -101,13 +102,13 @@
       __builtin_memcpy(&data_crc, h + 12 + len[r], 4);
       bool ok = mask_crc(crc32c_sw(h, 8, 0, tab)) == len_crc &&
                 mask_crc(payload_crc) == data_crc;
-      if (!ok) atomicMin(crc_err, (unsigned long long)(r + 1));
+      if (!ok) atomicMin(crc_err, (unsigned long long)(rec_base + r + 1));
     } else {
       rc = scan_record(data, off[r], len[r], fmt, schema, st);
     }
-    if (rc != ERR_OK) set_err(err, rc, r);
+    if (rc != ERR_OK) set_err(err, rc, rec_base + r);
     for (int f = 0; f < F; ++f)
-      if (st[f].err != ERR_OK) set_err(err, st[f].err, r);
+      if (st[f].err != ERR_OK) set_err(err, st[f].err, rec_base + r);
   }
 }
 
@@ -128,12 +129,13 @@
 __global__ void extract_fields_kernel(const u8* __restrict__ data, i64 R, int F,
                                       const FieldStat* __restrict__ stats,
                                       const DevFieldDst* __restrict__ metas,
-                                      int32_t* __restrict__ err) {
+                                      int32_t* __restrict__ err, i64 r0) {
   i64 total = R * F;
   for (i64 idx = blockIdx.x * (i64)blockDim.x + threadIdx.x; idx < total;
        idx += (i64)gridDim.x * blockDim.x) {
-    i64 r = idx / F;
-    int f = (int)(idx - r * F);
+    i64 q = idx / F;
+    int f = (int)(idx - q * F);
+    i64 r = r0 + q;
     const DevFieldDst& m = metas[f];
     const FieldStat& st = stats[r * F + f];
     DecodeDst dst{m.i64_vals, m.f32_vals, m.bytes_data, m.elem_len, m.sub_count};
@@ -445,7 +447,8 @@
                                          const u8* __restrict__ schema_blob,
                                          int F, FieldStat* __restrict__ stats,
                                          int32_t* __restrict__ err,
-                                         unsigned long long* crc_err) {
+                                         unsigned long long* crc_err,
+                                         i64 rec_base) {
   __shared__ uint32_t tab[8][256];
   stage_crc_tables(tab);
   SchemaView schema = schema_view(schema_blob);
@@ -457,9 +460,9 @@
       FieldStat* st = stats + r * F;
       for (int f = 0; f < F; ++f) field_stat_clear(&st[f]);
       int32_t rc = scan_record(data, off[r], len[r], fmt, schema, st);
-      if (rc != ERR_OK) set_err(err, rc, r);
+      if (rc != ERR_OK) set_err(err, rc, rec_base + r);
       for (int f = 0; f < F; ++f)
-        if (st[f].err != ERR_OK) set_err(err, st[f].err, r);
+        if (st[f].err != ERR_OK) set_err(err, st[f].err, rec_base + r);
     }
     if (crc_err) {
       const u8* h = data + off[r] - 12;
@@ -470,7 +473,7 @@
         __builtin_memcpy(&data_crc, h + 12 + len[r], 4);
         bool ok = mask_crc(crc32c_sw(h, 8, 0, tab)) == len_crc &&
                   mask_crc(payload) == data_crc;
-        if (!ok) atomicMin(crc_err, (unsigned long long)(r + 1));
+        if (!ok) atomicMin(crc_err, (unsigned long long)(rec_base + r + 1));
       }
     }
   }
@@ -480,13 +483,14 @@
                                            int F,
                                            const FieldStat* __restrict__ stats,
                                            const DevFieldDst* __restrict__ metas,
-                                           int32_t* __restrict__ err) {
+                                           int32_t* __restrict__ err, i64 r0) {
   i64 total = R * F;
   i64 wave = (blockIdx.x * (i64)blockDim.x + threadIdx.x) / 64;
   i64 nwaves = ((i64)gridDim.x * blockDim.x) / 64;
   for (i64 idx = wave; idx < total; idx += nwaves) {
-    i64 r = idx / F;
-    int f = (int)(idx - r * F);
+    i64 q = idx / F;
+    int f = (int)(idx - q * F);
+    i64 r = r0 + q;
     const DevFieldDst& m = metas[f];
     const FieldStat& st = stats[r * F + f];
     DecodeDst dst{m.i64_vals, m.f32_vals, m.bytes_data, m.elem_len, m.sub_count};
@@ -791,6 +795,22 @@
                        cand_len[slot] = len;
                        ++slot;
                      });
+}
+
+__global__ void frame_chain_kernel(const i64* __restrict__ pos,
+                                   const i64* __restrict__ len, i64 C,
+                                   const i64* __restrict__ carry_in,
+                                   i64* __restrict__ carry_out,
+                                   i64* __restrict__ off,
+                                   i64* __restrict__ broken) {
+  for (i64 k = blockIdx.x * (i64)blockDim.x + threadIdx.x; k < C;
+       k += (i64)gridDim.x * blockDim.x) {
+    i64 p = pos[k];
+    i64 want = k == 0 ? *carry_in : pos[k - 1] + 16 + len[k - 1];
+    if (p != want) *broken = 1;
+    off[k] = p + 12;
+    if (k == C - 1) *carry_out = p + 16 + len[k];
+  }
 }
 
 
@@ -1031,9 +1051,10 @@
 }
 
 
-inline int grid_for(i64 n) {
+inline int grid_for(i64 n, i64 max_blocks = 0) {
   i64 blocks = (n + kBlock - 1) / kBlock;
-  if (blocks > 8192) blocks = 8192;
+  i64 cap = max_blocks > 0 && max_blocks < 8192 ? max_blocks : 8192;
+  if (blocks > cap) blocks = cap;
   if (blocks < 1) blocks = 1;
   return (int)blocks;
 }
@@ -1056,26 +1077,30 @@
 void gpu_scan_records(uintptr_t data, uintptr_t off, uintptr_t len, i64 R,
                       int32_t fmt, uintptr_t schema_blob, int F, uintptr_t stats,
                       uintptr_t err, uintptr_t crc_err, uintptr_t stream,
-                      i64 avg_bytes) {
+                      i64 avg_bytes, i64 rec_base, i64 max_blocks) {
+  if (R <= 0) return;
   if (avg_bytes > kWaveRecordBytes) {
-    hipLaunchKernelGGL(scan_records_wave_kernel, dim3(grid_for(R * 64)),
+    hipLaunchKernelGGL(scan_records_wave_kernel,
+                       dim3(grid_for(R * 64, max_blocks)), dim3(kBlock), 0,
+                       (hipStream_t)stream, (const u8*)data, (const i64*)off,
+                       (const i64*)len, R, fmt, (const u8*)schema_blob, F,
+                       (FieldStat*)stats, (int32_t*)err,
+                       (unsigned long long*)crc_err, rec_base);
+  } else {
+    hipLaunchKernelGGL(scan_records_kernel, dim3(grid_for(R, max_blocks)),
                        dim3(kBlock), 0, (hipStream_t)stream, (const u8*)data,
                        (const i64*)off, (const i64*)len, R, fmt,
                        (const u8*)schema_blob, F, (FieldStat*)stats,
-                       (int32_t*)err, (unsigned long long*)crc_err);
-  } else {
-    hipLaunchKernelGGL(scan_records_kernel, dim3(grid_for(R)), dim3(kBlock), 0,
-                       (hipStream_t)stream, (const u8*)data, (const i64*)off,
-                       (const i64*)len, R, fmt, (const u8*)schema_blob, F,
-                       (FieldStat*)stats, (int32_t*)err,
-                       (unsigned long long*)crc_err);
+                       (int32_t*)err, (unsigned long long*)crc_err, rec_base);
   }
   HIP_CHECK(hipGetLastError());
 }
 
 void gpu_extract_fields(uintptr_t data, i64 R, int F, uintptr_t stats,
                         py::list metas, uintptr_t meta_dev, uintptr_t err,
-                        uintptr_t stream, i64 avg_bytes) {
+                        uintptr_t stream, i64 avg_bytes, i64 r0,
+                        i64 max_blocks) {
+  if (R <= 0 || F <= 0) return;
   std::vector<DevFieldDst> host_metas(F);
   for (int f = 0; f < F; ++f) {
     py::dict d = metas[f].cast<py::dict>();
@@ -1095,15 +1120,17 @@
                            sizeof(DevFieldDst) * F, hipMemcpyHostToDevice,
                            (hipStream_t)stream));
   if (avg_bytes > kWaveRecordBytes) {
-    hipLaunchKernelGGL(extract_fields_wave_kernel, dim3(grid_for(R * F * 64)),
-                       dim3(kBlock), 0, (hipStream_t)stream, (const u8*)data,
-                       R, F, (const FieldStat*)stats,
-                       (const DevFieldDst*)meta_dev, (int32_t*)err);
+    hipLaunchKernelGGL(extract_fields_wave_kernel,
+                       dim3(grid_for(R * F * 64, max_blocks)), dim3(kBlock), 0,
+                       (hipStream_t)stream, (const u8*)data, R, F,
+                       (const FieldStat*)stats, (const DevFieldDst*)meta_dev,
+                       (int32_t*)err, r0);
   } else {
-    hipLaunchKernelGGL(extract_fields_kernel, dim3(grid_for(R * F)),
-                       dim3(kBlock), 0, (hipStream_t)stream, (const u8*)data,
-                       R, F, (const FieldStat*)stats,
-                       (const DevFieldDst*)meta_dev, (int32_t*)err);
+    hipLaunchKernelGGL(extract_fields_kernel,
+                       dim3(grid_for(R * F, max_blocks)), dim3(kBlock), 0,
+                       (hipStream_t)stream, (const u8*)data, R, F,
+                       (const FieldStat*)stats, (const DevFieldDst*)meta_dev,
+                       (int32_t*)err, r0);
   }
   HIP_CHECK(hipGetLastError());
 }
@@ -1208,6 +1235,17 @@
   HIP_CHECK(hipGetLastError());
 }
 
+void gpu_frame_chain(uintptr_t pos, uintptr_t len, i64 C, uintptr_t carry_in,
+                     uintptr_t carry_out, uintptr_t off, uintptr_t broken,
+                     uintptr_t stream) {
+  if (C <= 0) return;
+  hipLaunchKernelGGL(frame_chain_kernel, dim3(grid_for(C)), dim3(kBlock), 0,
+                     (hipStream_t)stream, (const i64*)pos, (const i64*)len, C,
+                     (const i64*)carry_in, (i64*)carry_out, (i64*)off,
+                     (i64*)broken);
+  HIP_CHECK(hipGetLastError());
+}
+
 void gpu_infer_codes(uintptr_t data, uintptr_t off, uintptr_t len, i64 R,
                      int32_t fmt, uintptr_t table, int nslots, uintptr_t err,
                      uintptr_t stream) {
@@ -1266,13 +1304,20 @@
 
 struct Seg3Load {
   const i64* stats;
-  i64 R;
+  i64 n;
   int F;
+  i64 r0;
+  i64 stride;
+  const i64* b0;
+  const i64* b1;
+  const i64* b2;
   __host__ __device__ Seg3 operator()(i64 idx) const {
-    i64 f = idx / R;
-    i64 r = idx - f * R;
-    const i64* st = stats + (r * F + f) * 6;
-    return Seg3{st[2], st[3], st[4], r == 0 ? 1u : 0u};
+    i64 f = idx / n;
+    i64 q = idx - f * n;
+    const i64* st = stats + ((r0 + q) * F + f) * 6;
+    if (q != 0) return Seg3{st[2], st[3], st[4], 0u};
+    i64 at = f * stride + r0;
+    return Seg3{st[2] + b0[at], st[3] + b1[at], st[4] + b2[at], 1u};
   }
 };
 
@@ -1297,18 +1342,20 @@
   i64* b0;
   i64* b1;
   i64* b2;
-  i64 R;
+  i64 n;
+  i64 r0;
+  i64 stride;
   i64 pos;
   __host__ __device__ Seg3OutRef operator*() const { return (*this)[0]; }
   __host__ __device__ Seg3OutRef operator[](i64 k) const {
     i64 idx = pos + k;
-    i64 f = idx / R;
-    i64 r = idx - f * R;
-    i64 at = f * (R + 1) + r + 1;
+    i64 f = idx / n;
+    i64 q = idx - f * n;
+    i64 at = f * stride + r0 + q + 1;
     return Seg3OutRef{b0 + at, b1 + at, b2 + at};
   }
   __host__ __device__ Seg3OutIt operator+(i64 k) const {
-    return Seg3OutIt{b0, b1, b2, R, pos + k};
+    return Seg3OutIt{b0, b1, b2, n, r0, stride, pos + k};
   }
   __host__ __device__ Seg3OutIt& operator+=(i64 k) {
     pos += k;
@@ -1323,8 +1370,9 @@
 size_t gpu_stat_scan_temp_bytes(i64 R, int F) {
   size_t bytes = 0;
   auto in = rocprim::make_transform_iterator(
-      rocprim::make_counting_iterator<i64>(0), Seg3Load{nullptr, R, F});
-  Seg3OutIt out{nullptr, nullptr, nullptr, R, 0};
+      rocprim::make_counting_iterator<i64>(0),
+      Seg3Load{nullptr, R, F, 0, R + 1, nullptr, nullptr, nullptr});
+  Seg3OutIt out{nullptr, nullptr, nullptr, R, 0, R + 1, 0};
   (void)rocprim::inclusive_scan(nullptr, bytes, in, out, (size_t)(R * F),
                                 Seg3Combine());
   return bytes;
@@ -1332,16 +1380,24 @@
 
 void gpu_stat_scans(uintptr_t temp, size_t temp_bytes, uintptr_t stats, i64 R,
                     int F, uintptr_t val_base, uintptr_t byte_base,
-                    uintptr_t list_base, uintptr_t stream) {
+                    uintptr_t list_base, uintptr_t stream, i64 r0, i64 r1,
+                    i64 stride) {
   auto s = (hipStream_t)stream;
-  if (R <= 0 || F <= 0) return;
+  if (r1 < 0) r1 = R;
+  if (stride <= 0) stride = R + 1;
+  if (r0 < 0 || r1 > R || r1 >= stride)
+    throw std::runtime_error("gpu_stat_scans: range outside the planes");
+  i64 n = r1 - r0;
+  if (n <= 0 || F <= 0) return;
   auto in = rocprim::make_transform_iterator(
       rocprim::make_counting_iterator<i64>(0),
-      Seg3Load{(const i64*)stats, R, F});
-  Seg3OutIt out{(i64*)val_base, (i64*)byte_base, (i64*)list_base, R, 0};
+      Seg3Load{(const i64*)stats, n, F, r0, stride, (const i64*)val_base,
+               (const i64*)byte_base, (const i64*)list_base});
+  Seg3OutIt out{(i64*)val_base, (i64*)byte_base, (i64*)list_base, n, r0,
+                stride, 0};
   size_t tb = temp_bytes;
   HIP_CHECK(rocprim::inclusive_scan((void*)temp, tb, in, out,
-                                    (size_t)(R * F), Seg3Combine(), s));
+                                    (size_t)(n * F), Seg3Combine(), s));
 }
 
 void gpu_excl_sum_strided(uintptr_t temp, size_t temp_bytes, uintptr_t in,
@@ -1498,11 +1554,13 @@
   m.def("gpu_scan_records", &gpu_scan_records, py::arg("data"), py::arg("off"),
         py::arg("len"), py::arg("R"), py::arg("fmt"), py::arg("schema_blob"),
         py::arg("F"), py::arg("stats"), py::arg("err"), py::arg("crc_err"),
-        py::arg("stream"), py::arg("avg_bytes") = 0);
+        py::arg("stream"), py::arg("avg_bytes") = 0, py::arg("rec_base") = 0,
+        py::arg("max_blocks") = 0);
   m.def("gpu_extract_fields", &gpu_extract_fields, py::arg("data"),
         py::arg("R"), py::arg("F"), py::arg("stats"), py::arg("metas"),
         py::arg("meta_dev"), py::arg("err"), py::arg("stream"),
-        py::arg("avg_bytes") = 0);
+        py::arg("avg_bytes") = 0, py::arg("r0") = 0,
+        py::arg("max_blocks") = 0);
   m.def("gpu_size_records", &gpu_size_records);
   m.def("gpu_emit_records", &gpu_emit_records, py::arg("cols_dev"),
         py::arg("schema_blob"), py::arg("fmt"), py::arg("r0"), py::arg("R"),
@@ -1514,13 +1572,18 @@
   m.def("gpu_frame_scan_blocks", &gpu_frame_scan_blocks);
   m.def("gpu_frame_scan_count", &gpu_frame_scan_count);
   m.def("gpu_frame_scan_emit", &gpu_frame_scan_emit);
+  m.def("gpu_frame_chain", &gpu_frame_chain);
   m.def("gpu_gather_payloads", &gpu_gather_payloads, py::arg("data"),
         py::arg("off"), py::arg("len"), py::arg("dst_off"), py::arg("R"),
         py::arg("out"), py::arg("stream"), py::arg("avg_bytes") = 0);
   m.def("gpu_infer_codes", &gpu_infer_codes);
   m.def("gpu_scan_temp_bytes", &gpu_scan_temp_bytes);
   m.def("gpu_stat_scan_temp_bytes", &gpu_stat_scan_temp_bytes);
-  m.def("gpu_stat_scans", &gpu_stat_scans);
+  m.def("gpu_stat_scans", &gpu_stat_scans, py::arg("temp"),
+        py::arg("temp_bytes"), py::arg("stats"), py::arg("R"), py::arg("F"),
+        py::arg("val_base"), py::arg("byte_base"), py::arg("list_base"),
+        py::arg("stream"), py::arg("r0") = 0, py::arg("r1") = -1,
+        py::arg("stride") = 0);
   m.def("gpu_excl_sum_strided", &gpu_excl_sum_strided);
   m.def("file_mmap_pinned", &file_mmap_pinned, py::arg("path"), py::arg("n"),
         py::arg("writable"));
diff --git a/exp/exp_overlap.py b/exp/exp_overlap.py
--- /dev/null
+++ b/exp/exp_overlap.py
@@ -0,0 +1,108 @@
+import os
+import sys
+
+sys.path.insert(0, os.path.dirname(os.path.dirname(os.path.abspath(__file__))))
+import numpy as np
+import torch
+
+from bench import make_batch
+from spark_tfrecord_amd import _native
+from spark_tfrecord_amd.columnar import schema_blob, wire_fields
+from spark_tfrecord_amd.engine import gpu
+
+ROWS = int(os.environ.get("ROWS", 1_000_000))
+ROUNDS = int(os.environ.get("ROUNDS", 15))
+GRIDS = [int(g) for g in os.environ.get("GRIDS", "0,1024,256").split(",")]
+
+batch = make_batch(ROWS, seed=1234)
+path = "/dev/shm/exp_overlap.tfrecord"
+n = gpu.write_batch_to_file(gpu.batch_to_device(batch), path, "Example")
+ptr, pinned = _native.file_mmap_pinned(path, n, False)
+assert pinned, "needs a registered file mapping"
+
+data = gpu.read_file_to_device(path)
+off, lens = gpu.scan_frames_device(data)
+R = off.numel()
+ends = (off + lens + 4).cpu().numpy()
+fields = wire_fields(batch.schema)
+F = len(fields)
+blob = torch.frombuffer(bytearray(schema_blob(batch.schema)),
+                        dtype=torch.uint8).to("cuda")
+stats = torch.empty((R, F, 6), dtype=torch.int64, device="cuda")
+err = torch.zeros(2, dtype=torch.int32, device="cuda")
+crc_err = torch.full((1,), -1, dtype=torch.int64, device="cuda")
+avg = max(0, n // R - 16)
+
+span = gpu._READ_SLICE
+S = (n + span - 1) // span
+K = [int(np.searchsorted(ends, min(n, (s + 1) * span), side="right"))
+     for s in range(S)]
+main = torch.cuda.current_stream()
+streams = gpu._dma_streams()
+dst = torch.empty(n, dtype=torch.uint8, device="cuda")
+
+
+def scan(r0, r1, max_blocks):
+    if r1 <= r0:
+        return
+    _native.gpu_scan_records(dst.data_ptr(), off.data_ptr() + r0 * 8,
+                             lens.data_ptr() + r0 * 8, r1 - r0,
+                             gpu.FMT["Example"], blob.data_ptr(), F,
+                             stats.data_ptr() + r0 * F * 48, err.data_ptr(),
+                             crc_err.data_ptr(), main.cuda_stream, avg,
+                             rec_base=r0, max_blocks=max_blocks)
+
+
+def run(mode, max_blocks=0):
+    torch.cuda.synchronize()
+    t0 = torch.cuda.Event(enable_timing=True)
+    t_h2d = [torch.cuda.Event(enable_timing=True) for _ in streams]
+    t_end = torch.cuda.Event(enable_timing=True)
+    t0.record(main)
+    for st in streams:
+        st.wait_stream(main)
+    events = []
+    for s in range(S):
+        b0, b1 = s * span, min(n, (s + 1) * span)
+        st = streams[s % len(streams)]
+        _native.gpu_memcpy_h2d(dst.data_ptr() + b0, ptr + b0, b1 - b0,
+                               st.cuda_stream)
+        ev = torch.cuda.Event()
+        ev.record(st)
+        events.append(ev)
+    for st, e in zip(streams, t_h2d):
+        e.record(st)
+    done = 0
+    for s in range(S):
+        main.wait_event(events[s])
+        if mode == "ovl":
+            scan(done, K[s], max_blocks)
+            done = K[s]
+    if mode == "serial":
+        scan(0, R, 0)
+    t_end.record(main)
+    torch.cuda.synchronize()
+    return max(t0.elapsed_time(e) for e in t_h2d), t0.elapsed_time(t_end)
+
+
+variants = [("h2d", "h2d", 0), ("serial", "serial", 0)] + \
+    [(f"ovl@{g}", "ovl", g) for g in GRIDS]
+for _, mode, g in variants:
+    run(mode, g)
+res = {name: [] for name, _, _ in variants}
+for _ in range(ROUNDS):
+    for name, mode, g in variants:
+        res[name].append(run(mode, g))
+assert int(crc_err.item()) == -1 and int(err[0].item()) == 0
+
+print(f"# {n / 1e6:.1f} MB, {R} records, {S} slices of {span >> 20} MiB, "
+      f"{ROUNDS} rounds; ms from first copy issue")
+print(f"{'variant':10s} {'h2d med':>8s} {'h2d min-max':>15s} "
+      f"{'end med':>8s} {'end min-max':>15s}")
+for name, _, _ in variants:
+    a = np.asarray(res[name])
+    print(f"{name:10s} {np.median(a[:, 0]):8.3f} "
+          f"{a[:, 0].min():7.3f}-{a[:, 0].max():7.3f} "
+          f"{np.median(a[:, 1]):8.3f} "
+          f"{a[:, 1].min():7.3f}-{a[:, 1].max():7.3f}")
+os.unlink(path)
diff --git a/spark_tfrecord_amd/engine/gpu.py b/spark_tfrecord_amd/engine/gpu.py
--- a/spark_tfrecord_amd/engine/gpu.py
+++ b/spark_tfrecord_amd/engine/gpu.py
@@ -8,6 +8,7 @@
 import torch
 
 from .. import _native
+from . import stream_plan
 from ..columnar import RecordBatch, WireColumn, schema_blob, wire_fields
 from ..schema import KIND_BYTES, KIND_FLOAT, KIND_INT64, StructType, is_sequence_field, wire_kind_of
 
@@ -56,9 +57,13 @@
 
 
 _CHUNK = 64 << 20
-_READ_SLICE = int(os.environ.get("TFREC_READ_SLICE", 48 << 20))
+_READ_SLICE = int(os.environ.get("TFREC_READ_SLICE", 32 << 20))
+_SPLIT_SLICES = os.environ.get("TFREC_READ_SPLIT", "1") != "0"
 _WRITE_SLICES = int(os.environ.get("TFREC_WRITE_SLICES", 8))
-_PRESCAN = os.environ.get("TFREC_PRESCAN", "0") == "1"
+_STREAM_DECODE = os.environ.get("TFREC_STREAM_DECODE", "1") != "0"
+_STREAM_HEADROOM = float(os.environ.get("TFREC_STREAM_HEADROOM", 1.125))
+_STREAM_MAX_BLOCKS = int(os.environ.get("TFREC_STREAM_MAX_BLOCKS", 0))
+_STREAM_EXTRACT = os.environ.get("TFREC_STREAM_EXTRACT", "1") != "0"
 _SYNC_WRITES = os.environ.get("TFREC_SYNC", "1") != "0"
 
 
@@ -200,6 +205,16 @@
                                  out_ptr, n, _stream())
 
 
+def _stat_scan_workspace(R: int, F: int, device) -> torch.Tensor:
+    key = ("stat", device.index if hasattr(device, "index") else 0)
+    need = _native.gpu_stat_scan_temp_bytes(R, F)
+    ws = _scan_ws.get(key)
+    if ws is None or ws.numel() < need:
+        ws = torch.empty(int(need * 2) or 1, dtype=torch.uint8, device=device)
+        _scan_ws[key] = ws
+    return ws
+
+
 def excl_sum(t: torch.Tensor) -> torch.Tensor:
     n = t.numel()
     out = torch.empty(n + 1, dtype=torch.int64, device=t.device)
@@ -237,45 +252,6 @@
                                  block_counts.data_ptr(), _stream())
     off, lens, _ = _emit_and_chain(data, [(0, N)], block_counts, N)
     return off, lens
-
-
-def _prescan_prefix(data, pre_ranges, block_counts, nblocks, N, arrived,
-                    schema, record_type):
-    device = data.device
-    nb_pre = sum(nblocks[:len(pre_ranges)])
-    if nb_pre == 0:
-        return None
-    block_off = excl_sum(block_counts[:nb_pre])
-    C = int(block_off[-1].item())
-    if C == 0:
-        return None
-    pos = torch.empty(C, dtype=torch.int64, device=device)
-    lens = torch.empty(C, dtype=torch.int64, device=device)
-    base = 0
-    for s, e in pre_ranges:
-        _native.gpu_frame_scan_emit(data.data_ptr(), N, s, e, base,
-                                    block_off.data_ptr(), pos.data_ptr(),
-                                    lens.data_ptr(), _stream())
-        base += _native.gpu_frame_scan_blocks(s, e)
-    K = int(torch.searchsorted(pos + 16 + lens, torch.tensor(
-        arrived + 1, device=device)).item())
-    if K == 0:
-        return None
-    fields = wire_fields(schema)
-    F = len(fields)
-    if F == 0:
-        return None
-    blob = torch.frombuffer(bytearray(schema_blob(schema)),
-                            dtype=torch.uint8).to(device)
-    stats1 = torch.empty((K, F, 6), dtype=torch.int64, device=device)
-    err1 = torch.zeros(2, dtype=torch.int32, device=device)
-    off1 = (pos[:K] + 12).contiguous()
-    lens1 = lens[:K].contiguous()
-    _native.gpu_scan_records(data.data_ptr(), off1.data_ptr(),
-                             lens1.data_ptr(), K, FMT[record_type],
-                             blob.data_ptr(), F, stats1.data_ptr(),
-                             err1.data_ptr(), 0, _stream())
-    return stats1, err1, K
 
 
 def _emit_and_chain(data, ranges, block_counts, N):
@@ -336,7 +312,7 @@
 
 def decode_device(data: torch.Tensor, off: torch.Tensor, lens: torch.Tensor,
                   schema: StructType, record_type: str,
-                  verify_crc: bool = True, prescan=None) -> RecordBatch:
+                  verify_crc: bool = True) -> RecordBatch:
     check_native()
     device = data.device
     R = off.numel()
@@ -367,39 +343,19 @@
                 for f in fields]
         return RecordBatch(schema, cols, R)
 
-    blob = torch.frombuffer(bytearray(schema_blob(schema)),
-                            dtype=torch.uint8).to(device)
+    blob = _schema_blob_device(schema, device)
     stats = torch.empty((R, F, 6), dtype=torch.int64, device=device)
     err = torch.zeros(2, dtype=torch.int32, device=device)
     crc_err = None
     fuse_crc = verify_crc
     if fuse_crc:
         crc_err = torch.full((1,), -1, dtype=torch.int64, device=device)
-    r0 = 0
-    err1 = None
-    if prescan is not None:
-        stats1, err1, K = prescan
-        if K <= R and stats1.shape[1] == F:
-            stats[:K].copy_(stats1)
-            r0 = K
-        else:
-            err1 = None
     avg_bytes = max(0, (data.numel() // R) - 16) if R else 0
-    if R > r0:
-        stride = F * 6 * 8
-        _native.gpu_scan_records(data.data_ptr(), off.data_ptr() + r0 * 8,
-                                 lens.data_ptr() + r0 * 8, R - r0,
-                                 FMT[record_type], blob.data_ptr(), F,
-                                 stats.data_ptr() + r0 * stride,
-                                 err.data_ptr(),
-                                 crc_err.data_ptr() if fuse_crc else 0,
-                                 _stream(), avg_bytes)
-    crc_err_pre = None
-    if fuse_crc and r0 > 0:
-        crc_err_pre = torch.full((1,), -1, dtype=torch.int64, device=device)
-        _native.gpu_crc_verify(data.data_ptr(), off.data_ptr(),
-                               lens.data_ptr(), r0, crc_err_pre.data_ptr(),
-                               _stream(), 0)
+    _native.gpu_scan_records(data.data_ptr(), off.data_ptr(), lens.data_ptr(),
+                             R, FMT[record_type], blob.data_ptr(), F,
+                             stats.data_ptr(), err.data_ptr(),
+                             crc_err.data_ptr() if fuse_crc else 0,
+                             _stream(), avg_bytes)
 
     val_base = torch.empty((F, R + 1), dtype=torch.int64, device=device)
     byte_base = torch.empty((F, R + 1), dtype=torch.int64, device=device)
@@ -407,45 +363,65 @@
     val_base[:, 0] = 0
     byte_base[:, 0] = 0
     list_base[:, 0] = 0
-    key = ("stat", device.index if hasattr(device, "index") else 0)
-    need = _native.gpu_stat_scan_temp_bytes(R, F)
-    ws = _scan_ws.get(key)
-    if ws is None or ws.numel() < need:
-        ws = torch.empty(int(need * 2) or 1, dtype=torch.uint8, device=device)
-        _scan_ws[key] = ws
+    ws = _stat_scan_workspace(R, F, device)
     _native.gpu_stat_scans(ws.data_ptr(), ws.numel(), stats.data_ptr(), R, F,
                            val_base.data_ptr(), byte_base.data_ptr(),
                            list_base.data_ptr(), _stream())
     totals = torch.stack([val_base[:, -1], byte_base[:, -1], list_base[:, -1]])
     totals_h = totals.cpu()
-    if fuse_crc:
-        bad = int(crc_err.item())
-        bad_abs = (bad - 1 + r0) if bad != -1 else -1
-        if crc_err_pre is not None:
-            bp = int(crc_err_pre.item())
-            if bp != -1:
-                bad_abs = bp - 1 if bad_abs == -1 else min(bad_abs, bp - 1)
-        if bad_abs != -1:
-            raise RuntimeError(
-                f"corrupt TFRecord: bad CRC in record {bad_abs}")
-    rc = int(err[0].item())
-    rec = int(err[1].item()) - 1 + r0
-    if rc == 0 and err1 is not None:
-        rc = int(err1[0].item())
-        rec = int(err1[1].item()) - 1
+    _raise_scan_errors(int(crc_err.item()) if fuse_crc else -1,
+                       int(err[0].item()), int(err[1].item()))
+    cols = _extract_columns(data, R, fields, stats, val_base, byte_base,
+                            list_base, totals_h, err, avg_bytes)
+    if int(err[0].item()) != 0:
+        _raise_extract_error(int(err[0].item()), int(err[1].item()))
+    return RecordBatch(schema, cols, R)
+
+
+_schema_blobs = {}
+
+
+def _schema_blob_device(schema: StructType, device) -> torch.Tensor:
+    raw = bytes(schema_blob(schema))
+    key = (raw, str(torch.device(device)))
+    blob = _schema_blobs.get(key)
+    if blob is None:
+        if len(_schema_blobs) >= 64:
+            _schema_blobs.clear()
+        blob = torch.frombuffer(bytearray(raw), dtype=torch.uint8).to(device)
+        _schema_blobs[key] = blob
+    return blob
+
+
+def _raise_scan_errors(crc_bad: int, rc: int, rec1: int):
+    if crc_bad != -1:
+        raise RuntimeError(f"corrupt TFRecord: bad CRC in record {crc_bad - 1}")
     if rc != 0:
+        rec = rec1 - 1
         where = f" in record {rec}" if rec >= 0 else ""
         raise RuntimeError(f"TFRecord decode failed{where} (native error "
                            f"{rc}; kind mismatch or malformed record)")
 
+
+def _raise_extract_error(rc: int, rec1: int):
+    rec = rec1 - 1
+    where = f" (record {rec})" if rec >= 0 else ""
+    raise RuntimeError(f"TFRecord decode failed in value extraction"
+                       f"{where} (native error {rc})")
+
+
+def _extract_columns(data, R, fields, stats, val_base, byte_base, list_base,
+                     totals_h, err, avg_bytes) -> List[WireColumn]:
+    device = data.device
+    F = len(fields)
     metas = []
     outs = []
     for i, f in enumerate(fields):
         kind = wire_kind_of(f.dataType)
         seq = is_sequence_field(f.dataType)
-        nv = int(totals_h[0, i])
-        nb = int(totals_h[1, i])
-        nl = int(totals_h[2, i])
+        nv = int(totals_h[0][i])
+        nb = int(totals_h[1][i])
+        nl = int(totals_h[2][i])
         o = {"kind": kind, "seq": seq}
         o["i64_vals"] = torch.empty(nv if kind == KIND_INT64 else 0,
                                     dtype=torch.int64, device=device)
@@ -489,12 +465,7 @@
                   o["f32_vals"] if kind == KIND_FLOAT else o["bytes_data"])
         cols.append(WireColumn(kind, seq, presence, val_base[i], values,
                                elem_off, list_base[i] if seq else None, sub_off))
-    if int(err[0].item()) != 0:
-        rec = int(err[1].item()) - 1
-        where = f" (record {rec})" if rec >= 0 else ""
-        raise RuntimeError(f"TFRecord decode failed in value extraction"
-                           f"{where} (native error {int(err[0].item())})")
-    return RecordBatch(schema, cols, R)
+    return cols
 
 
 def decode_buffer_device(data_np: np.ndarray, schema: StructType, record_type: str,
@@ -630,6 +601,9 @@
     return total
 
 
+last_read = {}
+
+
 def read_file_to_batch_pipelined(path: str, schema: StructType, record_type: str,
                                  verify_crc: bool = True,
                                  device="cuda") -> RecordBatch:
@@ -648,17 +622,11 @@
         off, lens = scan_frames_device(data)
         return decode_device(data, off, lens, schema, record_type, verify_crc)
     data = torch.empty(n, dtype=torch.uint8, device=device)
-    span = _READ_SLICE
-    S = max(1, (n + span - 1) // span)
-    ranges = []
-    scanned = 0
-    for s in range(S):
-        b1 = min(n, (s + 1) * span)
-        scan_end = b1 - 32 if s < S - 1 else n
-        if scan_end > scanned:
-            ranges.append((scanned, scan_end))
-            scanned = scan_end
-    nblocks = [int(_native.gpu_frame_scan_blocks(a, b)) for a, b in ranges]
+    device = data.device
+    plan = stream_plan.plan_slices(n, _READ_SLICE)
+    S = len(plan)
+    nblocks = [int(_native.gpu_frame_scan_blocks(p.scan_lo, p.scan_hi))
+               if p.scan_hi > p.scan_lo else 0 for p in plan]
     block_counts = torch.empty(max(sum(nblocks), 1), dtype=torch.int64,
                                device=device)
     main = torch.cuda.current_stream()
@@ -666,54 +634,313 @@
     events = []
     for st in streams:
         st.wait_stream(main)
-    for s in range(S):
-        b0, b1 = s * span, min(n, (s + 1) * span)
-        st = streams[s % len(streams)]
-        _native.gpu_memcpy_h2d(data.data_ptr() + b0, ptr + b0, b1 - b0,
-                               st.cuda_stream)
-        ev = torch.cuda.Event()
-        ev.record(st)
-        events.append(ev)
+    for s, p in enumerate(plan):
+        half = (p.b1 - p.b0) // 2 if _SPLIT_SLICES and len(streams) > 1 else 0
+        parts = ([(p.b0, p.b0 + half, 0), (p.b0 + half, p.b1, 1)] if half
+                 else [(p.b0, p.b1, s % len(streams))])
+        evs = []
+        for lo, hi, k in parts:
+            st = streams[k]
+            _native.gpu_memcpy_h2d(data.data_ptr() + lo, ptr + lo, hi - lo,
+                                   st.cuda_stream)
+            ev = torch.cuda.Event()
+            ev.record(st)
+            evs.append(ev)
+        events.append(evs)
     data.record_stream(streams[0])
     if len(streams) > 1:
         data.record_stream(streams[1])
 
-    def launch_counts(ri: int, base: int):
-        _native.gpu_frame_scan_count(data.data_ptr(), n, ranges[ri][0],
-                                     ranges[ri][1], base,
-                                     block_counts.data_ptr(), _stream())
-
-    k0 = ((2 * S) // 3 if _PRESCAN and S >= 3 and record_type != "ByteArray"
-          else 0)
-
-    ri = 0
+    fields = wire_fields(schema)
+    F = len(fields)
+    streaming = _STREAM_DECODE
+    last_read.update(path="streamed", slices=S, regrows=0)
+    do_scan = streaming and record_type != "ByteArray" and F > 0
+    fuse_crc = verify_crc
+    vals = None
+    if streaming:
+        status = torch.zeros(_ST_CARRY + 1 + S, dtype=torch.int64,
+                             device=device)
+        status[_ST_CRC] = -1
+        sp = status.data_ptr()
+        err = status[_ST_ERR:_ST_ERR + 1].view(torch.int32)
+        xerr = status[_ST_XERR:_ST_XERR + 1].view(torch.int32)
+        rows = _StreamRows(n, F if do_scan else 0, device)
+        if do_scan:
+            blob = _schema_blob_device(schema, device)
+            vals = _StreamValues(fields, n, device) if _STREAM_EXTRACT else None
+            meta_dev = torch.empty(F * _native.gpu_devmeta_bytes(),
+                                   dtype=torch.uint8, device=device)
+
     base = 0
-
-    def consume_slices(upto: int):
-        nonlocal ri, base
-        for s in range(upto):
-            if events[s] is None:
+    C = 0
+    nchain = 0
+    r_done = 0
+    pending = None
+    avg_bytes = None
+    for s, p in enumerate(plan):
+        for ev in events[s]:
+            main.wait_event(ev)
+        last = s == S - 1
+        nb = nblocks[s]
+        if nb:
+            _native.gpu_frame_scan_count(data.data_ptr(), n, p.scan_lo,
+                                         p.scan_hi, base,
+                                         block_counts.data_ptr(), _stream())
+        if not streaming:
+            base += nb
+            continue
+        if nb:
+            block_off = excl_sum(block_counts[base:base + nb])
+            c_s = int(block_off[-1].item())
+            base += nb
+            if c_s:
+                rows.reserve(C + c_s, C, r_done, p.scan_hi)
+                _native.gpu_frame_scan_emit(
+                    data.data_ptr(), n, p.scan_lo, p.scan_hi, 0,
+                    block_off.data_ptr(), rows.pos.data_ptr() + C * 8,
+                    rows.lens.data_ptr() + C * 8, _stream())
+                _native.gpu_frame_chain(
+                    rows.pos.data_ptr() + C * 8, rows.lens.data_ptr() + C * 8,
+                    c_s, sp + (_ST_CARRY + nchain) * 8,
+                    sp + (_ST_CARRY + 1 + nchain) * 8,
+                    rows.off.data_ptr() + C * 8, sp + _ST_BROKEN * 8, _stream())
+                nchain += 1
+                C += c_s
+        if not do_scan or C == r_done:
+            continue
+        if last:
+            avail = C
+            end = n
+        else:
+            st_h = status.cpu()
+            if int(st_h[_ST_BROKEN]) != 0:
+                streaming = do_scan = False
                 continue
-            main.wait_event(events[s])
-            events[s] = None
-            scan_end = min(n, (s + 1) * span) - 32 if s < S - 1 else n
-            if ri < len(ranges) and ranges[ri][1] == scan_end:
-                launch_counts(ri, base)
-                base += nblocks[ri]
-                ri += 1
-
-    prescan = None
-    if k0:
-        consume_slices(k0)
-        prescan = _prescan_prefix(data, ranges[:ri], block_counts, nblocks, n,
-                                  arrived=min(n, k0 * span), schema=schema,
-                                  record_type=record_type)
-    consume_slices(S)
-    off, lens, clean = _emit_and_chain(data, ranges, block_counts, n)
-    if not clean:
-        prescan = None
-    return decode_device(data, off, lens, schema, record_type, verify_crc,
-                         prescan=prescan)
+            end = int(st_h[_ST_CARRY + nchain])
+            avail = stream_plan.arrived_records(C, end, p.b1)
+            if avail < C:
+                end = p.b1
+        if avail > r_done:
+            if avg_bytes is None:
+                avg_bytes = max(0, end // avail - 16)
+            _native.gpu_scan_records(
+                data.data_ptr(), rows.off.data_ptr() + r_done * 8,
+                rows.lens.data_ptr() + r_done * 8, avail - r_done,
+                FMT[record_type], blob.data_ptr(), F,
+                rows.stats.data_ptr() + r_done * F * 48, err.data_ptr(),
+                sp + _ST_CRC * 8 if fuse_crc else 0, _stream(), avg_bytes,
+                rec_base=r_done, max_blocks=0 if last else _STREAM_MAX_BLOCKS)
+            if vals is not None:
+                rows.scan_stats(r_done, avail)
+                if last:
+                    pending = (r_done, avail)
+                elif vals.ok:
+                    h = torch.cat(rows.totals(avail)
+                                  + [status[:_ST_CARRY]]).cpu()
+                    pair = h[3 * F + _ST_ERR:3 * F + _ST_ERR + 1].view(torch.int32)
+                    if int(h[3 * F + _ST_CRC]) != -1 or int(pair[0]) != 0:
+                        vals.ok = False
+                    else:
+                        vals.extract(data, rows, r_done, avail,
+                                     h[:3 * F].view(3, F), end, meta_dev,
+                                     xerr, avg_bytes,
+                                     _STREAM_MAX_BLOCKS)
+            r_done = avail
+
+    def unstreamed():
+        last_read["path"] = "fallback" if _STREAM_DECODE else "unstreamed"
+        ranges = [(p.scan_lo, p.scan_hi) for p in plan if p.scan_hi > p.scan_lo]
+        off, lens, _ = _emit_and_chain(data, ranges, block_counts, n)
+        return decode_device(data, off, lens, schema, record_type, verify_crc)
+
+    if not streaming or C == 0:
+        return unstreamed()
+    R = C
+    if not do_scan:
+        st_h = status.cpu()
+        if int(st_h[_ST_BROKEN]) != 0 or int(st_h[_ST_CARRY + nchain]) != n:
+            return unstreamed()
+        return decode_device(data, rows.off[:R], rows.lens[:R], schema,
+                             record_type, verify_crc)
+
+    stats = rows.stats[:R]
+    if vals is None:
+        rows.scan_stats(0, R)
+    packed = torch.cat(rows.totals(R) + [status]).cpu()
+    st_h = packed[3 * F:]
+    if int(st_h[_ST_BROKEN]) != 0 or int(st_h[_ST_CARRY + nchain]) != n:
+        return unstreamed()
+    pair = st_h[_ST_ERR:_ST_ERR + 1].view(torch.int32)
+    _raise_scan_errors(int(st_h[_ST_CRC]) if fuse_crc else -1, int(pair[0]),
+                       int(pair[1]))
+    totals_h = packed[:3 * F].view(3, F)
+    val_base, byte_base, list_base = rows.planes
+    if vals is None:
+        cols = _extract_columns(data, R, fields, stats,
+                                val_base[:, :R + 1], byte_base[:, :R + 1],
+                                list_base[:, :R + 1], totals_h, xerr,
+                                max(0, n // R - 16))
+    else:
+        if not vals.ok:
+            raise RuntimeError("streamed decode: scan error lost")
+        if pending is not None:
+            vals.extract(data, rows, pending[0], pending[1], totals_h, n,
+                         meta_dev, xerr, avg_bytes, 0)
+        cols = vals.columns(stats, val_base, list_base, R)
+    err_h = xerr.cpu()
+    if int(err_h[0]) != 0:
+        _raise_extract_error(int(err_h[0]), int(err_h[1]))
+    return RecordBatch(schema, cols, R)
+
+
+_ST_BROKEN, _ST_CRC, _ST_ERR, _ST_XERR, _ST_CARRY = 0, 1, 2, 3, 4
+
+
+class _StreamRows:
+
+    def __init__(self, total_bytes: int, F: int, device):
+        self.total_bytes = total_bytes
+        self.F = F
+        self.device = device
+        self.cap = 0
+        self.pos = self.lens = self.off = self.stats = None
+        self.planes = None
+
+    def _alloc(self, cap: int):
+        i64 = dict(dtype=torch.int64, device=self.device)
+        planes = None
+        if self.F:
+            planes = [torch.empty((self.F, cap + 1), **i64) for _ in range(3)]
+            for t in planes:
+                t[:, 0] = 0
+        return (torch.empty(cap, **i64), torch.empty(cap, **i64),
+                torch.empty(cap, **i64),
+                torch.empty((cap, self.F, 6), **i64) if self.F else None,
+                planes)
+
+    def scan_stats(self, r0: int, r1: int):
+        ws = _stat_scan_workspace(r1 - r0, self.F, self.device)
+        v, b, l = self.planes
+        _native.gpu_stat_scans(ws.data_ptr(), ws.numel(),
+                               self.stats.data_ptr(), r1, self.F, v.data_ptr(),
+                               b.data_ptr(), l.data_ptr(), _stream(), r0=r0,
+                               r1=r1, stride=self.cap + 1)
+
+    def totals(self, r: int) -> list:
+        return [t[:, r] for t in self.planes]
+
+    def reserve(self, need: int, n_cand: int, n_scanned: int, bytes_seen: int):
+        cap = stream_plan.grown_capacity(self.cap, need, bytes_seen,
+                                         self.total_bytes, _STREAM_HEADROOM)
+        if cap == self.cap:
+            return
+        pos, lens, off, stats, planes = self._alloc(cap)
+        if n_cand:
+            pos[:n_cand].copy_(self.pos[:n_cand])
+            lens[:n_cand].copy_(self.lens[:n_cand])
+            off[:n_cand].copy_(self.off[:n_cand])
+        if n_scanned and stats is not None:
+            stats[:n_scanned].copy_(self.stats[:n_scanned])
+            for new, old in zip(planes, self.planes):
+                new[:, :n_scanned + 1].copy_(old[:, :n_scanned + 1])
+        self.pos, self.lens, self.off, self.stats = pos, lens, off, stats
+        self.planes = planes
+        if self.cap:
+            last_read["regrows"] = last_read.get("regrows", 0) + 1
+        self.cap = cap
+
+
+class _StreamValues:
+
+    _DIMS = (("i64_vals", 0), ("f32_vals", 0), ("elem_len", 0),
+             ("bytes_data", 1), ("sub_count", 2))
+
+    def __init__(self, fields, total_bytes: int, device):
+        self.total_bytes = total_bytes
+        self.device = device
+        self.ok = True
+        self.kinds = [wire_kind_of(f.dataType) for f in fields]
+        self.seqs = [is_sequence_field(f.dataType) for f in fields]
+        self.filled = [[0] * len(fields) for _ in range(3)]
+        self.bufs = []
+        for kind in self.kinds:
+            dt = {"i64_vals": torch.int64, "f32_vals": torch.float32,
+                  "elem_len": torch.int64, "bytes_data": torch.uint8,
+                  "sub_count": torch.int64}
+            self.bufs.append({k: torch.empty(0, dtype=d, device=device)
+                              for k, d in dt.items()})
+
+    def _used(self, i: int, name: str) -> bool:
+        kind = self.kinds[i]
+        return {"i64_vals": kind == KIND_INT64, "f32_vals": kind == KIND_FLOAT,
+                "elem_len": kind == KIND_BYTES}.get(name, True)
+
+    def _reserve(self, totals, bytes_seen: int):
+        for i, bufs in enumerate(self.bufs):
+            for name, dim in self._DIMS:
+                if not self._used(i, name):
+                    continue
+                need = int(totals[dim][i])
+                old = bufs[name]
+                cap = stream_plan.grown_capacity(
+                    old.numel(), need, bytes_seen, self.total_bytes,
+                    _STREAM_HEADROOM, min_unit=1)
+                if cap == old.numel():
+                    continue
+                new = torch.empty(cap, dtype=old.dtype, device=self.device)
+                k = self.filled[dim][i]
+                if k:
+                    new[:k].copy_(old[:k])
+                if old.numel():
+                    last_read["regrows"] = last_read.get("regrows", 0) + 1
+                bufs[name] = new
+
+    def extract(self, data, rows, r0: int, r1: int, totals, bytes_seen: int,
+                meta_dev, xerr, avg_bytes: int, max_blocks: int):
+        self._reserve(totals, bytes_seen)
+        v, b, l = rows.planes
+        metas = []
+        for i, bufs in enumerate(self.bufs):
+            metas.append({
+                "kind": self.kinds[i], "is_seq": 1 if self.seqs[i] else 0,
+                "i64_vals": bufs["i64_vals"].data_ptr(),
+                "f32_vals": bufs["f32_vals"].data_ptr(),
+                "bytes_data": bufs["bytes_data"].data_ptr(),
+                "elem_len": bufs["elem_len"].data_ptr(),
+                "sub_count": bufs["sub_count"].data_ptr(),
+                "val_base": v[i].data_ptr(),
+                "byte_base": b[i].data_ptr(),
+                "list_base": l[i].data_ptr() if self.seqs[i] else 0,
+            })
+        _native.gpu_extract_fields(data.data_ptr(), r1 - r0, len(self.bufs),
+                                   rows.stats.data_ptr(), metas,
+                                   meta_dev.data_ptr(), xerr.data_ptr(),
+                                   _stream(), avg_bytes, r0=r0,
+                                   max_blocks=max_blocks)
+        self.filled = [[int(totals[d][i]) for i in range(len(self.bufs))]
+                       for d in range(3)]
+
+    def columns(self, stats, val_base, list_base, R: int) -> List[WireColumn]:
+        cols = []
+        for i, bufs in enumerate(self.bufs):
+            kind, seq = self.kinds[i], self.seqs[i]
+            nv, nb, nl = (self.filled[d][i] for d in range(3))
+            presence = (stats[:, i, 0] >= 0).to(torch.uint8)
+            elem_off = None
+            if kind == KIND_BYTES:
+                elem_off = excl_sum(bufs["elem_len"][:nv])
+            sub_off = None
+            if seq:
+                sub_off = excl_sum(bufs["sub_count"][:nl])
+            values = (bufs["i64_vals"][:nv] if kind == KIND_INT64 else
+                      bufs["f32_vals"][:nv] if kind == KIND_FLOAT else
+                      bufs["bytes_data"][:nb])
+            cols.append(WireColumn(kind, seq, presence, val_base[i][:R + 1],
+                                   values, elem_off,
+                                   list_base[i][:R + 1] if seq else None,
+                                   sub_off))
+        return cols
 
 
 def gz_device_meta(path: str):
diff --git a/spark_tfrecord_amd/engine/stream_plan.py b/spark_tfrecord_amd/engine/stream_plan.py
--- /dev/null
+++ b/spark_tfrecord_amd/engine/stream_plan.py
@@ -0,0 +1,52 @@
+
+from __future__ import annotations
+
+from typing import List, NamedTuple
+
+MIN_FRAME = 16
+SCAN_LOOKAHEAD = 32
+
+
+class SlicePlan(NamedTuple):
+    b0: int
+    b1: int
+    scan_lo: int
+    scan_hi: int
+
+
+def plan_slices(n: int, span: int) -> List[SlicePlan]:
+    if n <= 0:
+        return []
+    span = max(1, int(span))
+    S = (n + span - 1) // span
+    out = []
+    scanned = 0
+    for s in range(S):
+        b0, b1 = s * span, min(n, (s + 1) * span)
+        hi = b1 - SCAN_LOOKAHEAD if s < S - 1 else n
+        hi = max(hi, scanned)
+        out.append(SlicePlan(b0, b1, scanned, hi))
+        scanned = hi
+    return out
+
+
+def arrived_records(n_cand: int, last_end: int, arrived: int) -> int:
+    if n_cand <= 0:
+        return 0
+    return n_cand if last_end <= arrived else n_cand - 1
+
+
+def row_capacity(need: int, bytes_seen: int, total_bytes: int,
+                 headroom: float, min_unit: int = MIN_FRAME) -> int:
+    need = max(int(need), 0)
+    bytes_seen = min(max(int(bytes_seen), 1), max(int(total_bytes), 1))
+    est = int(need * (total_bytes / bytes_seen) * max(headroom, 1.0)) + 1
+    most = need + max(total_bytes - bytes_seen, 0) // max(min_unit, 1)
+    return max(need, min(est, most), 1)
+
+
+def grown_capacity(cap: int, need: int, bytes_seen: int, total_bytes: int,
+                   headroom: float, min_unit: int = MIN_FRAME) -> int:
+    if need <= cap:
+        return cap
+    return row_capacity(need, bytes_seen, total_bytes, headroom, min_unit)
diff --git a/spark_tfrecord_amd/io/writer.py b/spark_tfrecord_amd/io/writer.py
--- a/spark_tfrecord_amd/io/writer.py
+++ b/spark_tfrecord_amd/io/writer.py
@@ -318,6 +318,11 @@
                 P.write_file_atomic(payload, fpath)
                 return len(payload)
 
+            owner = {}
+            for p, _, _ in ranges:
+                owner[tuple(_partition_dir_value(v) for v in combos[p])] = p
+            ranges = [r for r in ranges if owner[tuple(
+                _partition_dir_value(v) for v in combos[r[0]])] == r[0]]
             for nb in P.shared_pool().map(lambda a: _write_part(*a), ranges):
                 if metrics is not None:
                     metrics.add(nbytes=nb, files=1)
```
